# ppt0011/distributed_training

Hardware: AMD Instinct MI355X
Metric: images/sec (node) ResNet-50 at 1/2/4/8 MI355X; grad-sync bus GB/s (higher is better)
Workload: dtype bf16

## Files before the change

distributed_training_amd/_lib.py:

```python
from __future__ import annotations

import ctypes
import os
import threading

import torch

LIB_PATH = os.environ.get(
    "GSYNC_LIB", os.path.join(os.path.dirname(os.path.abspath(__file__)), "lib", "libgsync.so")
)

GS_OK = 0
GS_EINVAL, GS_EHIP, GS_ERCCL, GS_ESTATE, GS_ENOMEM, GS_ENODEV = -1, -2, -3, -4, -5, -6
GS_F32, GS_BF16, GS_F16, GS_F64, GS_I64, GS_I32, GS_U8 = 0, 1, 2, 3, 4, 5, 6
GS_DEV_HOST, GS_DEV_HIP = 0, 1
GS_SUM, GS_PROD, GS_MAX, GS_MIN, GS_AVG = 0, 1, 2, 3, 4
GS_SCALE_NONE, GS_SCALE_MUL, GS_SCALE_DIV = 0, 1, 2
GS_PLAN_SLOTS = 5
GS_RED_GROUPS = 64
GS_RED_PARTIALS = 1024
GS_BKT_AUTO_COLLECTIVE = 1
GS_BKT_GRAD_VIEW = 2
GS_BKT_NO_SCALE = 4
GS_BKT_REDUCE_SCATTER = 8
GS_BKT_NO_UNPACK = 16
GS_LAYOUT_NCHW, GS_LAYOUT_NHWC = 0, 1
GS_OP_PACK, GS_OP_UNPACK, GS_OP_SCALE, GS_OP_SQNORM, GS_OP_UNSCALE, GS_OP_SGD, GS_OP_ADAM, GS_OP_SUM = 1, 2, 3, 4, 5, 6, 7, 8
GS_OP_LARS_NORM, GS_OP_LARS = 9, 10
GS_OP_LAMB_MOMENTS, GS_OP_LAMB = 11, 12
GS_OP_EMA = 13
GS_EMA_EMA, GS_EMA_SWA, GS_EMA_WARMUP = 0, 1, 2

_TORCH_TO_GS = {
    torch.float32: GS_F32,
    torch.bfloat16: GS_BF16,
    torch.float16: GS_F16,
    torch.float64: GS_F64,
    torch.int64: GS_I64,
    torch.int32: GS_I32,
    torch.uint8: GS_U8,
}

_c_int, _c_i64, _c_f, _c_d, _vp = ctypes.c_int, ctypes.c_int64, ctypes.c_float, ctypes.c_double, ctypes.c_void_p
_p_i64 = ctypes.POINTER(ctypes.c_int64)
_p_i32 = ctypes.POINTER(ctypes.c_int32)
_p_u8 = ctypes.POINTER(ctypes.c_uint8)
_p_vp = ctypes.POINTER(ctypes.c_void_p)
_p_f = ctypes.POINTER(ctypes.c_float)

SIGNATURES = {
    "gs_version": (_c_int, []),
    "gs_last_error": (ctypes.c_char_p, []),
    "gs_device_count": (_c_int, []),
    "gs_set_host_threads": (_c_int, [_c_int]),
    "gs_comm_unique_id_bytes": (_c_int, []),
    "gs_comm_get_unique_id": (_c_int, [_p_u8]),
    "gs_comm_create": (_c_int, [_c_int, _c_int, _p_u8, _c_int, _p_vp]),
    "gs_comm_create_ex": (_c_int, [_c_int, _c_int, _p_u8, _c_int, _c_int, _p_vp]),
    "gs_comm_destroy": (_c_int, [_vp]),
    "gs_comm_abort": (_c_int, [_vp]),
    "gs_comm_set_timeout": (_c_int, [_vp, _c_i64]),
    "gs_comm_status": (_c_int, [_vp, ctypes.c_char_p, _c_int]),
    "gs_comm_rank": (_c_int, [_vp]),
    "gs_comm_world": (_c_int, [_vp]),
    "gs_comm_stream": (_c_int, [_vp, _p_vp]),
    "gs_stream_wait": (_c_int, [_vp, _vp]),
    "gs_allreduce": (_c_int, [_vp, _vp, _vp, _c_i64, _c_int, _c_int, _vp]),
    "gs_reduce_scatter": (_c_int, [_vp, _vp, _vp, _c_i64, _c_int, _c_int, _vp]),
    "gs_all_gather": (_c_int, [_vp, _vp, _vp, _c_i64, _c_int, _vp]),
    "gs_broadcast": (_c_int, [_vp, _vp, _vp, _c_i64, _c_int, _c_int, _vp]),
    "gs_allreduce_marked": (_c_int, [_vp, _vp, _vp, _c_i64, _c_int, _c_int, _vp, _vp]),
    "gs_all_gather_marked": (_c_int, [_vp, _vp, _vp, _c_i64, _c_int, _vp, _vp]),
    "gs_plan_create": (_c_int, [_c_int, _c_int, _c_int, _p_i64, _c_i64, _p_vp]),
    "gs_plan_create_ex": (_c_int, [_c_int, _c_int, _c_int, _p_i64, _c_i64, _c_i64, _p_vp]),
    "gs_plan_destroy": (_c_int, [_vp]),
    "gs_plan_flat_numel": (_c_i64, [_vp]),
    "gs_plan_offsets": (_c_int, [_vp, _p_i64]),
    "gs_plan_n_tasks": (_c_int, [_vp]),
    "gs_plan_task_units": (_c_i64, [_vp]),
    "gs_plan_set_hyper_source": (_c_int, [_vp, _vp]),
    "gs_watchdog_pause": (_c_int, [_c_int]),
    "gs_adam_hyper": (_c_int, [_c_int, _vp, _vp, _c_d, _c_d, _c_d, _vp, _vp, _vp]),
    "gs_plan_timer_enable": (_c_int, [_vp, _c_int]),
    "gs_plan_timer_read": (_c_int, [_vp, _p_f, _p_i32, _c_int]),
    "gs_plan_set_ptrs": (_c_int, [_vp, _c_int, _p_vp, _vp]),
    "gs_pack": (_c_int, [_vp, _c_int, _c_int, _vp, _c_int, _c_f, _c_int, _vp]),
    "gs_unpack": (_c_int, [_vp, _vp, _c_int, _c_int, _c_int, _vp, _c_int, _vp]),
    "gs_unpack_check": (_c_int, [_vp, _vp, _c_int, _c_int, _c_int, _vp, _vp]),
    "gs_scale": (_c_int, [_vp, _c_int, _c_int, _c_f, _c_int, _vp]),
    "gs_sqnorm": (_c_int, [_vp, _c_int, _c_int, _vp, _c_int, _vp]),
    "gs_sum": (_c_int, [_vp, _c_int, _c_int, _vp, _c_int, _vp]),
    "gs_sqnorm_partial": (_c_int, [_vp, _c_int, _c_int, _vp]),
    "gs_plan_set_clip": (_c_int, [_vp, _vp, _c_f, _c_f, _c_f, _c_f, _vp]),
    "gs_plan_set_read_hint": (_c_int, [_vp, _c_int]),
    "gs_sqnorm_partial_out": (_c_int, [_vp, _c_int, _c_int, _vp, _p_i32, _vp]),
    "gs_plan_set_clip_groups": (_c_int, [_vp, _vp, ctypes.c_int32, _c_f, _c_f, _c_f, _c_f, _vp]),
    "gs_clip_scale": (_c_int, [_vp, _c_int, _c_int, _vp]),
    "gs_rng_state_bytes": (_c_int, []),
    "gs_rng_draw_u32": (_c_int, [_vp, _c_i64, _c_i64, _vp]),
    "gs_randperm": (_c_int, [ctypes.c_uint64, _c_i64, _vp]),
    "gs_distributed_sampler_indices": (_c_int, [_c_i64, _c_int, _c_int, _c_int, ctypes.c_uint64, _c_i64, _c_int,
                                                _vp, _c_i64, _p_i64]),
    "gs_crop_flip_params": (_c_int, [_vp, _c_i64, _c_int, _c_int, _c_int, _c_int, _c_int, _c_int, _vp, _c_i64,
                                     _vp]),
    "gs_image_augment": (_c_int, [_c_int, _c_int, _vp, _vp, _c_i64, _c_int, _c_int, _c_int, _c_int, _c_int, _c_int,
                                  _vp, _c_i64, _vp, _c_int, _c_int, _vp, _vp]),
    "gs_bn_bwd_partials": (_c_int, [_c_i64, _c_int]),
    "gs_bn_bwd_reduce": (_c_int, [_vp, _vp, _vp, _vp, _vp, _vp, _c_i64, _c_i64, _c_int, _vp]),
    "gs_bn_bwd_reduce_fork": (_c_int, [_vp, _vp, _vp, _vp, _vp, _vp, _vp, _c_i64, _c_i64, _c_int, _vp]),
    "gs_bn_bwd_dx": (_c_int, [_vp, _vp, _vp, _vp, _vp, _vp, _vp, _c_i64, _vp, _vp, _vp, _c_i64, _c_int, _vp]),
    "gs_add_relu_fwd": (_c_int, [_vp, _vp, _c_i64, _vp]),
    "gs_relu_maxpool_fwd": (_c_int, [_vp, _vp, _vp, _c_i64, _c_int, _c_int, _c_int, _vp]),
    "gs_maxpool_bwd": (_c_int, [_vp, _vp, _vp, _vp, _c_i64, _c_int, _c_int, _c_int, _vp]),
    "gs_bn_infer_act": (_c_int, [_vp, _vp, _vp, _vp, _vp, _vp, _c_d, _c_int, _vp, _c_i64, _c_int, _vp]),
    "gs_bn_infer_relu_maxpool": (_c_int, [_vp, _vp, _vp, _vp, _vp, _c_d, _vp, _c_i64, _c_int, _c_int, _c_int, _vp]),
    "gs_eval_accumulate": (_c_int, [_c_int, _vp, _c_int, _vp, _c_i64, _c_i64, _c_i64, _c_i64, _p_i32, _c_int, _c_i64,
                                    _vp, _vp, _vp]),
    "gs_clip_coef":(_c_int, [_c_int, _vp, _c_f, _c_f, _vp, _vp, _vp]),
    "gs_unscale_check": (_c_int, [_vp, _c_int, _c_int, _vp, _vp, _vp]),
    "gs_sgd_step": (
        _c_int,
        [_vp, _c_int, _c_int, _c_d, _c_d, _c_d, _c_d, _c_int, _c_int, _c_int, _vp, _vp, _vp],
    ),
    "gs_adam_step": (
        _c_int,
        [_vp, _c_int, _c_int, _c_d, _c_d, _c_d, _c_d, _c_d, _c_int, _c_int, _c_d, _c_d, _vp, _vp, _vp],
    ),
    "gs_plan_set_adapt": (_c_int, [_vp, _p_i32]),
    "gs_lars_norms": (_c_int, [_vp, _c_int, _vp, _vp]),
    "gs_lars_step": (_c_int, [_vp, _c_int, _c_d, _c_d, _c_d, _c_d, _c_d, _vp, _vp, _vp, _vp]),
    "gs_lars_step_lowp": (_c_int, [_vp, _c_int, _c_int, _c_d, _c_d, _c_d, _c_d, _c_d, _vp, _vp, _vp, _vp]),
    "gs_lamb_step_lowp": (_c_int, [_vp, _c_int, _c_d, _c_d, _c_d, _c_d, _c_d, _c_d, _c_d, _vp, _vp, _vp]),
    "gs_lamb_moments": (_c_int, [_vp, _c_int, _c_d, _c_d, _c_d, _c_d, _c_d, _c_d, _vp, _vp, _vp, _vp]),
    "gs_lamb_step": (_c_int, [_vp, _c_d, _c_d, _c_d, _c_d, _c_d, _c_d, _c_d, _vp, _vp, _vp]),
    "gs_lamb_hyper": (_c_int, [_c_int, _vp, _vp, _c_d, _c_d, _c_int, _vp, _vp, _vp]),
    "gs_ema_step": (_c_int, [_vp, _c_int, _c_int, _c_d, _c_int, _vp]),
    "gs_ema_hyper": (_c_int, [_c_int, _vp, _c_int, _c_d, _vp, _vp]),
    "gs_compute_bucket_assignment": (
        _c_int,
        [_c_int, _p_i64, _p_i32, _p_i32, _c_int, _p_i64, _p_i32, _p_i32, _p_i32],
    ),
    "gs_bucketer_create": (
        _c_int,
        [_vp, _c_int, _c_int, _c_int, _p_i64, _c_int, _c_int, _p_i32, _p_i32, _c_int, _c_i64, _c_f, _c_int, _p_vp],
    ),
    "gs_bucketer_destroy": (_c_int, [_vp]),
    "gs_bucketer_bucket_numel": (_c_int, [_vp, _c_int, _p_i64]),
    "gs_bucketer_shard_numel": (_c_int, [_vp, _c_int, _p_i64]),
    "gs_bucketer_param_location": (_c_int, [_vp, _c_int, _p_i32, _p_i64]),
    "gs_bucketer_set_bucket_buffer": (_c_int, [_vp, _c_int, _vp]),
    "gs_bucketer_set_shard_buffer": (_c_int, [_vp, _c_int, _vp]),
    "gs_bucketer_prepare": (_c_int, [_vp, _vp]),
    "gs_bucketer_mark_ready": (_c_int, [_vp, _c_int, _vp, _vp, _p_i32, _p_i32]),
    "gs_bucketer_mark_unused": (_c_int, [_vp, _vp, _p_i32, _p_i32]),
    "gs_bucketer_finalize": (_c_int, [_vp, _vp]),
    "gs_bucketer_unpack_bucket": (_c_int, [_vp, _c_int, _vp]),
    "gs_bucketer_set_found_inf": (_c_int, [_vp, _vp]),
    "gs_bucketer_set_div_factor": (_c_int, [_vp, _c_f]),
    "gs_bucketer_set_debug": (_c_int, [_vp, _vp]),
    "gs_bucketer_set_bucket_dtype": (_c_int, [_vp, _c_int, _c_int, _c_int]),
    "gs_bucketer_last_comm_ms": (_c_int, [_vp, _c_int, _p_f]),
    "gs_bucketer_last_timing": (_c_int, [_vp, _c_int, _p_f]),
    "gs_bucketer_set_timeline": (_c_int, [_vp, _c_int]),
    "gs_bucketer_bucket_stream": (_c_int, [_vp, _c_int, ctypes.POINTER(_vp)]),
    "gs_bucketer_set_mark_consumer": (_c_int, [_vp, _vp]),
    "gs_bucketer_first_pack_plan": (_c_int, [_vp, _p_vp]),
}


class GsyncError(RuntimeError):
    """A libgsync entry point returned an error (message from gs_last_error)."""


class GsyncUnavailable(GsyncError):
    """libgsync.so is missing or failed to load."""


_lock = threading.Lock()
_lib = None
_load_error: str | None = None


def _load():
    global _lib, _load_error
    with _lock:
        if _lib is not None or _load_error is not None:
            return
        if not os.path.exists(LIB_PATH):
            _load_error = (
                f"libgsync not built: {LIB_PATH} is missing "
                "(run `python -c 'import __graft_entry__ as g; g.build()'` or `make -C distributed_training_amd/csrc`)"
            )
            return
        try:
            lib = ctypes.CDLL(LIB_PATH)
        except OSError as e:
            _load_error = f"failed to load {LIB_PATH}: {e}"
            return
        for name, (res, args) in SIGNATURES.items():
            fn = getattr(lib, name)
            fn.restype = res
            fn.argtypes = args
        _lib = lib


def lib():
    if _lib is None:
        _load()
        if _lib is None:
            raise GsyncUnavailable(_load_error)
    return _lib


def available() -> bool:
    try:
        lib()
        return True
    except GsyncUnavailable:
        return False


HOOK_PATH = os.path.join(os.path.dirname(os.path.abspath(LIB_PATH)), "_gshook.so")
if not os.path.exists(HOOK_PATH):
    HOOK_PATH = os.path.join(os.path.dirname(os.path.abspath(__file__)), "lib", "_gshook.so")
_hook_mod = None
_hook_error: str | None = None


def hook_module():
    global _hook_mod, _hook_error
    if _hook_mod is not None or _hook_error is not None:
        return _hook_mod
    lib()
    if os.path.realpath(LIB_PATH) != os.path.realpath(os.path.join(os.path.dirname(HOOK_PATH), "libgsync.so")):
        _hook_error = f"GSYNC_LIB={LIB_PATH} is not the library _gshook links"
        return None
    if not os.path.exists(HOOK_PATH):
        _hook_error = f"{HOOK_PATH} is not built"
        return None
    import importlib.util

    spec = importlib.util.spec_from_file_location("_gshook", HOOK_PATH)
    mod = importlib.util.module_from_spec(spec)
    spec.loader.exec_module(mod)
    _hook_mod = mod
    return mod


def check(rc: int, what: str = "") -> int:
    if rc < 0:
        msg = lib().gs_last_error().decode(errors="replace")
        raise GsyncError(f"{what or 'libgsync'} failed ({rc}): {msg}")
    return rc


def gs_dtype(dtype: torch.dtype) -> int:
    try:
        return _TORCH_TO_GS[dtype]
    except KeyError:
        raise TypeError(f"libgsync: unsupported dtype {dtype}") from None


def device_kind(t: torch.Tensor) -> int:
    if t.device.type == "cuda":
        return GS_DEV_HIP
    if t.device.type == "cpu":
        return GS_DEV_HOST
    raise TypeError(f"libgsync: unsupported device {t.device}")


def i64_array(vals):
    arr = (ctypes.c_int64 * max(1, len(vals)))(*vals)
    return arr


def i32_array(vals):
    return (ctypes.c_int32 * max(1, len(vals)))(*vals)


def ptr_array(vals):
    return (ctypes.c_void_p * max(1, len(vals)))(*vals)


def stream_ptr(device: torch.device) -> int | None:
    if device.type != "cuda":
        return None
    return torch.cuda.current_stream(device).cuda_stream


_deferred: list = []


def _capturing() -> bool:
    try:
        return torch.cuda.is_available() and torch.cuda.is_current_stream_capturing()
    except Exception:
        return False


def destroy(fn_name: str, handle) -> None:
    if _capturing():
        _deferred.append((fn_name, handle))
        return
    getattr(lib(), fn_name)(handle)


def flush_deferred() -> None:
    if not _deferred or _capturing():
        return
    while _deferred:
        fn_name, h = _deferred.pop(0)
        getattr(lib(), fn_name)(h)
```

distributed_training_amd/csrc/gs_bn_kernels.hip:

```cpp
#include <hip/hip_runtime.h>

#include <algorithm>
#include <climits>
#include <cmath>

#include "gs_common.h"

#ifndef GS_BN_NT
#define GS_BN_NT 0
#endif
#ifndef GS_BN_DX_RNE
#define GS_BN_DX_RNE 0
#endif

namespace gs {
namespace {

#define HIP_RET(expr)                                                               \
  do {                                                                              \
    hipError_t _e = (expr);                                                         \
    if (_e != hipSuccess)                                                           \
      return fail(GS_EHIP, std::string(#expr " failed: ") + hipGetErrorString(_e)); \
  } while (0)

typedef uint32_t bu4 __attribute__((ext_vector_type(4)));
typedef float bf4 __attribute__((ext_vector_type(4)));

constexpr int kBnTileVecs = 8;
constexpr int kBnMaxP = 512;
constexpr int kBnTargetBlocks = 1024;
constexpr int kBnUnroll = 4;
#ifndef GS_BN_FORK_UNROLL
#define GS_BN_FORK_UNROLL 4
#endif
constexpr int kBnForkUnroll = GS_BN_FORK_UNROLL;

struct BnGeom {
  int tx_log2;
  int ctiles;
  int P;
  int64_t rpb;
};

BnGeom bn_geom(int64_t R, int C) {
  const int V = C / 8;
  int l2 = 0;
  while ((1 << l2) < V && (1 << l2) < kBnTileVecs) ++l2;
  const int tx = 1 << l2, ty = kBlock / tx;
  const int64_t ctiles = (V + tx - 1) / tx;
  int64_t P = std::min<int64_t>(kBnMaxP, (R + ty - 1) / ty);
  P = std::min<int64_t>(P, static_cast<int64_t>(std::sqrt(0.5 * static_cast<double>(R))));
  P = std::min<int64_t>(P, kBnTargetBlocks / ctiles);
  P = std::max<int64_t>(P, 1);
  if (ctiles * P > 256) {
    const int64_t step = 256 / std::min<int64_t>(256, ctiles & -ctiles);
    if (P >= step) P -= P % step;
  }
  const int64_t rpb = (R + P - 1) / P;
  P = (R + rpb - 1) / rpb;
  return BnGeom{l2, static_cast<int>(ctiles), static_cast<int>(P), rpb};
}

__device__ __forceinline__ uint32_t to_bf16(float f) {
  uint32_t u = __float_as_uint(f);
  if ((u & 0x7fffffffu) > 0x7f800000u) return 0x7FC0u;
  return (u + 0x7FFFu + ((u >> 16) & 1u)) >> 16;
}

__device__ __forceinline__ void unpack8(const bu4& v, float (&f)[8]) {
#pragma unroll
  for (int i = 0; i < 4; ++i) {
    f[2 * i] = __uint_as_float(v[i] << 16);
    f[2 * i + 1] = __uint_as_float(v[i] & 0xffff0000u);
  }
}

__device__ __forceinline__ bu4 pack8_exact(const float (&f)[8]) {
  bu4 v;
#pragma unroll
  for (int i = 0; i < 4; ++i) v[i] = (__float_as_uint(f[2 * i]) >> 16) | (__float_as_uint(f[2 * i + 1]) & 0xffff0000u);
  return v;
}

__device__ __forceinline__ uint32_t to_bf16_trunc(float f) {
  uint32_t u = __float_as_uint(f);
  if ((~u & 0x7f800000u) == 0 && (u & 0xffffu) != 0) u |= 0x10000u;
  return u >> 16;
}

__device__ __forceinline__ bu4 pack8_dx(const float (&f)[8]) {
  bu4 v;
#pragma unroll
  for (int i = 0; i < 4; ++i) {
    if constexpr (GS_BN_DX_RNE) v[i] = to_bf16(f[2 * i]) | (to_bf16(f[2 * i + 1]) << 16);
    else v[i] = to_bf16_trunc(f[2 * i]) | (to_bf16_trunc(f[2 * i + 1]) << 16);
  }
  return v;
}

template <bool NT>
__device__ __forceinline__ bu4 ld16(const uint16_t* p) {
  const bu4* q = reinterpret_cast<const bu4*>(p);
  if constexpr (NT) return __builtin_nontemporal_load(q);
  else return *q;
}

__device__ __forceinline__ void st16(uint16_t* p, const bu4& v) { *reinterpret_cast<bu4*>(p) = v; }

__device__ __forceinline__ void relu_mask(float (&g)[8], const bu4& yv) {
  float yf[8];
  unpack8(yv, yf);
#pragma unroll
  for (int i = 0; i < 8; ++i) g[i] = yf[i] <= 0.f ? 0.f : g[i];
}

__device__ __forceinline__ void fork_sum(float (&g)[8], const bu4& bv) {
  float b[8];
  unpack8(bv, b);
#pragma unroll
  for (int i = 0; i < 8; ++i) g[i] = __uint_as_float(to_bf16(g[i] + b[i]) << 16);
}

template <bool RELU, bool WRITE_G, bool FORK>
__global__ void __launch_bounds__(kBlock)
bn_bwd_reduce_kernel(const uint16_t* __restrict__ x, const uint16_t* __restrict__ dy, const uint16_t* __restrict__ dy2,
                     const uint16_t* __restrict__ y, uint16_t* __restrict__ gout, const float* __restrict__ mean,
                     float* __restrict__ ws, int64_t R, int C, int tx_log2, int64_t rpb) {
  constexpr int U = FORK ? kBnForkUnroll : kBnUnroll;
  __shared__ float s_red[kBlock * 16];
  __shared__ double s_grp[kBlock];
  const int t = threadIdx.x;
  const int tx = 1 << tx_log2, ty = kBlock >> tx_log2;
  const int tx_i = t & (tx - 1), ty_i = t >> tx_log2;
  const int v = blockIdx.x * tx + tx_i;
  const bool active = v < (C >> 3);
  const int c0 = v * 8;
  const int64_t r0 = static_cast<int64_t>(blockIdx.y) * rpb;
  const int64_t r1 = std::min<int64_t>(R, r0 + rpb);

  float sg[8], sq[8], m[8];
#pragma unroll
  for (int i = 0; i < 8; ++i) {
    sg[i] = 0.f;
    sq[i] = 0.f;
    m[i] = active ? mean[c0 + i] : 0.f;
  }
  auto body = [&](const bu4& xv, const bu4& dv, const bu4& bv, const bu4& yv, int64_t off) {
    float xf[8], g[8];
    unpack8(xv, xf);
    unpack8(dv, g);
    if constexpr (FORK) fork_sum(g, bv);
    if constexpr (RELU) relu_mask(g, yv);
    if constexpr (WRITE_G) st16(gout + off, pack8_exact(g));
#pragma unroll
    for (int i = 0; i < 8; ++i) {
      sg[i] += g[i];
      sq[i] = fmaf(g[i], xf[i] - m[i], sq[i]);
    }
  };
  if (active) {
    const int64_t step = static_cast<int64_t>(ty) * C;
    int64_t r = r0 + ty_i;
    int64_t off = r * C + c0;
    for (; r + (U - 1) * ty < r1; r += U * ty, off += U * step) {
      bu4 xv[U], dv[U], bv[U] = {}, yv[U] = {};
#pragma unroll
      for (int k = 0; k < U; ++k) {
        xv[k] = ld16<false>(x + off + k * step);
        dv[k] = ld16<GS_BN_NT && WRITE_G>(dy + off + k * step);
        if constexpr (FORK) bv[k] = ld16<GS_BN_NT>(dy2 + off + k * step);
        if constexpr (RELU) yv[k] = ld16<GS_BN_NT && WRITE_G>(y + off + k * step);
      }
#pragma unroll
      for (int k = 0; k < U; ++k) body(xv[k], dv[k], bv[k], yv[k], off + k * step);
    }
    for (; r < r1; r += ty, off += step) {
      bu4 bv = {0u, 0u, 0u, 0u}, yv = {0u, 0u, 0u, 0u};
      const bu4 xv = ld16<false>(x + off), dv = ld16<false>(dy + off);
      if constexpr (FORK) bv = ld16<false>(dy2 + off);
      if constexpr (RELU) yv = ld16<false>(y + off);
      body(xv, dv, bv, yv, off);
    }
  }
  const int F = 16 << tx_log2;
#pragma unroll
  for (int i = 0; i < 8; ++i) {
    s_red[t * 16 + 2 * i] = sg[i];
    s_red[t * 16 + 2 * i + 1] = sq[i];
  }
  __syncthreads();
  {
    const int o = t & (F - 1), grp = t >> (tx_log2 + 4);
    double a = 0.0;
#pragma unroll
    for (int k = 0; k < 16; ++k) a += static_cast<double>(s_red[(grp * 16 + k) * F + o]);
    s_grp[t] = a;
  }
  __syncthreads();
  if (t < F) {
    const int G = kBlock / F;
    double a = 0.0;
    for (int k = 0; k < G; ++k) a += s_grp[k * F + t];
    const int ch = blockIdx.x * (tx * 8) + (t >> 1);
    if (ch < C) ws[(static_cast<int64_t>(blockIdx.y) * C + ch) * 2 + (t & 1)] = static_cast<float>(a);
  }
}

template <bool RELU>
__global__ void __launch_bounds__(kBlock)
bn_bwd_dx_kernel(const uint16_t* __restrict__ x, const uint16_t* __restrict__ dy, const uint16_t* __restrict__ y,
                 const float* __restrict__ mean, const float* __restrict__ invstd, const float* __restrict__ weight,
                 const float* __restrict__ ws, int P, uint16_t* __restrict__ dx, float* __restrict__ gw,
                 float* __restrict__ gb, int64_t R, int C, int tx_log2, int64_t rpb, double inv_R) {
  __shared__ double s_fold[kBlock * 4];
  __shared__ double s_sum[16 * kBnTileVecs];
  const int t = threadIdx.x;
  const int tx = 1 << tx_log2, ty = kBlock >> tx_log2;
  const int tx_i = t & (tx - 1), ty_i = t >> tx_log2;
  const int tile_c0 = blockIdx.x * (tx * 8);
  {
    const int F4 = 4 << tx_log2, G4 = kBlock / F4;
    const int q = t & (F4 - 1), grp = t >> (tx_log2 + 2);
    double a[4] = {0.0, 0.0, 0.0, 0.0};
    if (tile_c0 + 2 * q < C) {
      const bf4* base = reinterpret_cast<const bf4*>(ws + static_cast<int64_t>(tile_c0) * 2) + q;
      const int64_t stride = C >> 1;
#pragma unroll 8
      for (int p = grp; p < P; p += G4) {
        const bf4 w4 = base[p * stride];
#pragma unroll
        for (int j = 0; j < 4; ++j) a[j] += static_cast<double>(w4[j]);
      }
    }
#pragma unroll
    for (int j = 0; j < 4; ++j) s_fold[t * 4 + j] = a[j];
    __syncthreads();
    if (t < 4 * F4) {
      double b = 0.0;
      for (int k = 0; k < G4; ++k) b += s_fold[k * 4 * F4 + t];
      s_sum[t] = b;
    }
    __syncthreads();
  }
  if (blockIdx.y == 0 && t < tx * 8 && tile_c0 + t < C) {
    gb[tile_c0 + t] = static_cast<float>(s_sum[2 * t]);
    gw[tile_c0 + t] = static_cast<float>(static_cast<double>(invstd[tile_c0 + t]) * s_sum[2 * t + 1]);
  }
  const int v = blockIdx.x * tx + tx_i;
  if (v >= (C >> 3)) return;
  const int c0 = v * 8;
  float m[8], a[8], m1[8], k2[8];
#pragma unroll
  for (int i = 0; i < 8; ++i) {
    const float is = invstd[c0 + i];
    m[i] = mean[c0 + i];
    a[i] = weight[c0 + i] * is;
    m1[i] = static_cast<float>(s_sum[tx_i * 16 + 2 * i] * inv_R);
    k2[i] = static_cast<float>(static_cast<double>(is) * is * s_sum[tx_i * 16 + 2 * i + 1] * inv_R);
  }
  auto body = [&](const bu4& xv, const bu4& dv, const bu4& yv, int64_t off) {
    float xf[8], g[8];
    unpack8(xv, xf);
    unpack8(dv, g);
    if constexpr (RELU) relu_mask(g, yv);
#pragma unroll
    for (int i = 0; i < 8; ++i) g[i] = a[i] * fmaf(m[i] - xf[i], k2[i], g[i] - m1[i]);
    st16(dx + off, pack8_dx(g));
  };
  const int64_t r0 = static_cast<int64_t>(blockIdx.y) * rpb;
  const int64_t r1 = std::min<int64_t>(R, r0 + rpb);
  const int64_t step = static_cast<int64_t>(ty) * C;
  int64_t r = r0 + ty_i;
  int64_t off = r * C + c0;
  for (; r + (kBnUnroll - 1) * ty < r1; r += kBnUnroll * ty, off += kBnUnroll * step) {
    bu4 xv[kBnUnroll], dv[kBnUnroll], yv[kBnUnroll] = {};
#pragma unroll
    for (int k = 0; k < kBnUnroll; ++k) {
      xv[k] = ld16<GS_BN_NT>(x + off + k * step);
      dv[k] = ld16<GS_BN_NT>(dy + off + k * step);
      if constexpr (RELU) yv[k] = ld16<GS_BN_NT>(y + off + k * step);
    }
#pragma unroll
    for (int k = 0; k < kBnUnroll; ++k) body(xv[k], dv[k], yv[k], off + k * step);
  }
  for (; r < r1; r += ty, off += step) {
    bu4 yv = {0u, 0u, 0u, 0u};
    const bu4 xv = ld16<false>(x + off), dv = ld16<false>(dy + off);
    if constexpr (RELU) yv = ld16<false>(y + off);
    body(xv, dv, yv, off);
  }
}

__global__ void __launch_bounds__(kBlock)
add_relu_fwd_kernel(uint16_t* __restrict__ t, const uint16_t* __restrict__ id, int64_t nvec) {
  const int64_t base = static_cast<int64_t>(blockIdx.x) * (kBlock * kBnUnroll) + threadIdx.x;
  bu4 a[kBnUnroll], b[kBnUnroll];
#pragma unroll
  for (int k = 0; k < kBnUnroll; ++k) {
    const int64_t i = base + k * kBlock;
    if (i < nvec) {
      a[k] = ld16<false>(t + i * 8);
      b[k] = ld16<false>(id + i * 8);
    }
  }
#pragma unroll
  for (int k = 0; k < kBnUnroll; ++k) {
    const int64_t i = base + k * kBlock;
    if (i < nvec) {
      float af[8], bf[8];
      unpack8(a[k], af);
      unpack8(b[k], bf);
#pragma unroll
      for (int j = 0; j < 8; ++j) {
        const float s = __uint_as_float(to_bf16(af[j] + bf[j]) << 16);
        af[j] = s != s ? s : fmaxf(s, 0.f);
      }
      st16(t + i * 8, pack8_exact(af));
    }
  }
}


__device__ __forceinline__ float relu1(float v) { return v > 0.f ? v : (v != v ? v : 0.f); }

__global__ void __launch_bounds__(kBlock)
relu_maxpool_fwd_kernel(const uint16_t* __restrict__ y, uint16_t* __restrict__ pooled, uint8_t* __restrict__ idx,
                        int64_t nvec, int H, int W, int OH, int OW, int V) {
  const int64_t i = static_cast<int64_t>(blockIdx.x) * kBlock + threadIdx.x;
  if (i >= nvec) return;
  const int cv = static_cast<int>(i % V);
  int64_t p = i / V;
  const int ow = static_cast<int>(p % OW);
  p /= OW;
  const int oh = static_cast<int>(p % OH);
  const int64_t n = p / OH;
  const int h0 = 2 * oh - 1, w0 = 2 * ow - 1;
  const int64_t C = static_cast<int64_t>(V) * 8;
  bu4 in[9];
  bool ok[9];
#pragma unroll
  for (int kh = 0; kh < 3; ++kh) {
#pragma unroll
    for (int kw = 0; kw < 3; ++kw) {
      const int ih = h0 + kh, iw = w0 + kw, k = 3 * kh + kw;
      ok[k] = ih >= 0 && ih < H && iw >= 0 && iw < W;
      in[k] = bu4{0u, 0u, 0u, 0u};
      if (ok[k]) in[k] = ld16<false>(y + ((n * H + ih) * W + iw) * C + cv * 8);
    }
  }
  float best[8];
  uint32_t code[8];
#pragma unroll
  for (int j = 0; j < 8; ++j) {
    best[j] = -INFINITY;
    code[j] = 0;
  }
#pragma unroll
  for (int k = 0; k < 9; ++k) {
    float f[8];
    unpack8(in[k], f);
#pragma unroll
    for (int j = 0; j < 8; ++j) {
      const float v = relu1(f[j]);
      const bool take = ok[k] && (v > best[j] || v != v);
      best[j] = take ? v : best[j];
      code[j] = take ? static_cast<uint32_t>(k) : code[j];
    }
  }
  st16(pooled + i * 8, pack8_exact(best));
  uint2 c;
  c.x = code[0] | (code[1] << 8) | (code[2] << 16) | (code[3] << 24);
  c.y = code[4] | (code[5] << 8) | (code[6] << 16) | (code[7] << 24);
  *reinterpret_cast<uint2*>(idx + i * 8) = c;
}

template <bool FORK>
__global__ void __launch_bounds__(kBlock)
maxpool_bwd_kernel(const uint16_t* __restrict__ da, const uint16_t* __restrict__ db, const uint8_t* __restrict__ idx,
                   uint16_t* __restrict__ dx, int64_t nquad, int H, int W, int OH, int OW, int V) {
  const int64_t i = static_cast<int64_t>(blockIdx.x) * kBlock + threadIdx.x;
  if (i >= nquad) return;
  const int cv = static_cast<int>(i % V);
  int64_t p = i / V;
  const int b = static_cast<int>(p % OW);
  p /= OW;
  const int a = static_cast<int>(p % OH);
  const int64_t n = p / OH;
  const bool more_h = a + 1 < OH, more_w = b + 1 < OW;
  uint2 cw[4];
  int64_t ovec[4];
  bool ok[4];
#pragma unroll
  for (int k = 0; k < 4; ++k) {
    const int al = k >> 1, be = k & 1;
    ok[k] = (al == 0 || more_h) && (be == 0 || more_w);
    ovec[k] = ((n * OH + a + al) * OW + b + be) * V + cv;
    cw[k] = uint2{0xffffffffu, 0xffffffffu};
    if (ok[k]) cw[k] = *reinterpret_cast<const uint2*>(idx + ovec[k] * 8);
  }
  auto has = [](const uint2& w, uint32_t c) {
    const uint32_t x0 = w.x ^ (c * 0x01010101u), x1 = w.y ^ (c * 0x01010101u);
    return ((((x0 - 0x01010101u) & ~x0) | ((x1 - 0x01010101u) & ~x1)) & 0x80808080u) != 0;
  };
  bool hit[4];
  hit[0] = true;
  hit[1] = ok[1] && (has(cw[1], 3u) || has(cw[1], 6u));
  hit[2] = ok[2] && (has(cw[2], 1u) || has(cw[2], 2u));
  hit[3] = ok[3] && has(cw[3], 0u);
  bu4 av[4], bv[4];
#pragma unroll
  for (int k = 0; k < 4; ++k) {
    av[k] = bv[k] = bu4{0u, 0u, 0u, 0u};
    if (hit[k]) {
      av[k] = ld16<false>(da + ovec[k] * 8);
      if constexpr (FORK) bv[k] = ld16<false>(db + ovec[k] * 8);
    }
  }
  const bool many = H * W > 1;
  float acc[4][8];
#pragma unroll
  for (int q = 0; q < 4; ++q)
#pragma unroll
    for (int j = 0; j < 8; ++j) acc[q][j] = 0.f;
#pragma unroll
  for (int k = 0; k < 4; ++k) {
    const int al = k >> 1, be = k & 1;
    float g[8];
    unpack8(av[k], g);
    if constexpr (FORK) fork_sum(g, bv[k]);
#pragma unroll
    for (int q = 0; q < 4; ++q) {
      const int dh = q >> 1, dw = q & 1;
      if (dh < al || dw < be) continue;
      const uint32_t want = static_cast<uint32_t>(3 * (dh + 1 - 2 * al) + (dw + 1 - 2 * be));
      const bool single = many && !(dh == 1 && more_h) && !(dw == 1 && more_w);
#pragma unroll
      for (int j = 0; j < 8; ++j) {
        const uint32_t cj = ((j < 4 ? cw[k].x : cw[k].y) >> (8 * (j & 3))) & 0xffu;
        const bool m = hit[k] && cj == want;
        acc[q][j] = m ? (single ? g[j] : acc[q][j] + g[j]) : acc[q][j];
      }
    }
  }
  const int64_t C = static_cast<int64_t>(V) * 8;
#pragma unroll
  for (int q = 0; q < 4; ++q) {
    const int ih = 2 * a + (q >> 1), iw = 2 * b + (q & 1);
    if (ih < H && iw < W) {
      bu4 out;
#pragma unroll
      for (int r = 0; r < 4; ++r) out[r] = to_bf16(acc[q][2 * r]) | (to_bf16(acc[q][2 * r + 1]) << 16);
      st16(dx + ((n * H + ih) * W + iw) * C + cv * 8, out);
    }
  }
}

constexpr int kBnInferBlocks = 2048;
#ifndef GS_BN_INFER_TILE_VECS
#define GS_BN_INFER_TILE_VECS 32
#endif
constexpr int kBnInferTileVecs = GS_BN_INFER_TILE_VECS;

BnGeom bn_infer_geom(int64_t R, int C) {
  const int V = C / 8;
  int l2 = 0;
  while ((1 << l2) < V && (1 << l2) < kBnInferTileVecs) ++l2;
  const int tx = 1 << l2, ty = kBlock / tx;
  const int64_t ctiles = (V + tx - 1) / tx;
  const int64_t per = static_cast<int64_t>(ty) * kBnUnroll;
  int64_t P = std::min<int64_t>((R + per - 1) / per, std::max<int64_t>(1, kBnInferBlocks / ctiles));
  P = std::max<int64_t>(P, 1);
  const int64_t rpb = (R + P - 1) / P;
  P = (R + rpb - 1) / rpb;
  return BnGeom{l2, static_cast<int>(ctiles), static_cast<int>(P), rpb};
}

__device__ __forceinline__ void infer_affine(const float* __restrict__ rm, const float* __restrict__ rv,
                                             const float* __restrict__ w, const float* __restrict__ b, float eps,
                                             int c0, float (&s)[8], float (&t)[8]) {
  const bf4 m0 = *reinterpret_cast<const bf4*>(rm + c0), m1 = *reinterpret_cast<const bf4*>(rm + c0 + 4);
  const bf4 v0 = *reinterpret_cast<const bf4*>(rv + c0), v1 = *reinterpret_cast<const bf4*>(rv + c0 + 4);
  const bf4 w0 = *reinterpret_cast<const bf4*>(w + c0), w1 = *reinterpret_cast<const bf4*>(w + c0 + 4);
  const bf4 b0 = *reinterpret_cast<const bf4*>(b + c0), b1 = *reinterpret_cast<const bf4*>(b + c0 + 4);
#pragma unroll
  for (int i = 0; i < 8; ++i) {
    const float m = i < 4 ? m0[i & 3] : m1[i & 3], v = i < 4 ? v0[i & 3] : v1[i & 3];
    const float wi = i < 4 ? w0[i & 3] : w1[i & 3], bi = i < 4 ? b0[i & 3] : b1[i & 3];
    s[i] = wi * (1.0f / sqrtf(v + eps));
    t[i] = fmaf(-m, s[i], bi);
  }
}

__device__ __forceinline__ bu4 pack8_rne(const float (&f)[8]) {
  bu4 v;
#pragma unroll
  for (int i = 0; i < 4; ++i) v[i] = to_bf16(f[2 * i]) | (to_bf16(f[2 * i + 1]) << 16);
  return v;
}

template <bool RES, bool RELU>
__global__ void __launch_bounds__(kBlock)
bn_infer_act_kernel(const uint16_t* x, const uint16_t* __restrict__ res, const float* __restrict__ rm,
                    const float* __restrict__ rv, const float* __restrict__ w, const float* __restrict__ b, float eps,
                    uint16_t* y, int64_t R, int C, int tx_log2, int64_t rpb) {
  const int t_ = threadIdx.x;
  const int tx = 1 << tx_log2, ty = kBlock >> tx_log2;
  const int tx_i = t_ & (tx - 1), ty_i = t_ >> tx_log2;
  const int v = blockIdx.x * tx + tx_i;
  if (v >= (C >> 3)) return;
  const int c0 = v * 8;
  const int64_t r0 = static_cast<int64_t>(blockIdx.y) * rpb;
  const int64_t r1 = std::min<int64_t>(R, r0 + rpb);
  const int64_t step = static_cast<int64_t>(ty) * C;
  int64_t r = r0 + ty_i;
  int64_t off = r * C + c0;
  float s[8], t[8];
  infer_affine(rm, rv, w, b, eps, c0, s, t);
  auto body = [&](const bu4& xv, const bu4& rvv, int64_t off) {
    float f[8], r[8];
    unpack8(xv, f);
    if constexpr (RES) unpack8(rvv, r);
#pragma unroll
    for (int i = 0; i < 8; ++i) {
      float a = fmaf(f[i], s[i], t[i]);
      if constexpr (RES) a = a + r[i];
      if constexpr (RELU) a = relu1(a);
      f[i] = a;
    }
    st16(y + off, pack8_rne(f));
  };
  for (; r + (kBnUnroll - 1) * ty < r1; r += kBnUnroll * ty, off += kBnUnroll * step) {
    bu4 xv[kBnUnroll], rr[kBnUnroll] = {};
#pragma unroll
    for (int k = 0; k < kBnUnroll; ++k) {
      xv[k] = ld16<GS_BN_NT>(x + off + k * step);
      if constexpr (RES) rr[k] = ld16<false>(res + off + k * step);
    }
#pragma unroll
    for (int k = 0; k < kBnUnroll; ++k) body(xv[k], rr[k], off + k * step);
  }
  for (; r < r1; r += ty, off += step) {
    bu4 rr = {0u, 0u, 0u, 0u};
    const bu4 xv = ld16<false>(x + off);
    if constexpr (RES) rr = ld16<false>(res + off);
    body(xv, rr, off);
  }
}

__global__ void __launch_bounds__(kBlock)
bn_infer_relu_maxpool_kernel(const uint16_t* __restrict__ x, const float* __restrict__ rm,
                             const float* __restrict__ rv, const float* __restrict__ w, const float* __restrict__ b,
                             float eps, uint16_t* __restrict__ pooled, int64_t OR, int H, int W, int OH, int OW, int C,
                             int tx_log2, int64_t rpb) {
  const int t_ = threadIdx.x;
  const int tx = 1 << tx_log2, ty = kBlock >> tx_log2;
  const int tx_i = t_ & (tx - 1), ty_i = t_ >> tx_log2;
  const int v = blockIdx.x * tx + tx_i;
  if (v >= (C >> 3)) return;
  const int c0 = v * 8;
  float s[8], t[8];
  infer_affine(rm, rv, w, b, eps, c0, s, t);
  const int64_t r0 = static_cast<int64_t>(blockIdx.y) * rpb;
  const int64_t r1 = std::min<int64_t>(OR, r0 + rpb);
  for (int64_t p = r0 + ty_i; p < r1; p += ty) {
    const int ow = static_cast<int>(p % OW);
    const int64_t q = p / OW;
    const int oh = static_cast<int>(q % OH);
    const int64_t n = q / OH;
    const int h0 = 2 * oh - 1, w0 = 2 * ow - 1;
    bu4 in[9];
    bool ok[9];
#pragma unroll
    for (int kh = 0; kh < 3; ++kh) {
#pragma unroll
      for (int kw = 0; kw < 3; ++kw) {
        const int ih = h0 + kh, iw = w0 + kw, k = 3 * kh + kw;
        ok[k] = ih >= 0 && ih < H && iw >= 0 && iw < W;
        in[k] = bu4{0u, 0u, 0u, 0u};
        if (ok[k]) in[k] = ld16<false>(x + ((n * H + ih) * W + iw) * C + c0);
      }
    }
    float best[8];
#pragma unroll
    for (int j = 0; j < 8; ++j) best[j] = -INFINITY;
#pragma unroll
    for (int k = 0; k < 9; ++k) {
      float f[8];
      unpack8(in[k], f);
#pragma unroll
      for (int j = 0; j < 8; ++j) {
        const float a = __uint_as_float(to_bf16(relu1(fmaf(f[j], s[j], t[j]))) << 16);
        const bool take = ok[k] && (a > best[j] || a != a);
        best[j] = take ? a : best[j];
      }
    }
    st16(pooled + p * C + c0, pack8_exact(best));
  }
}

bool aligned16(const void* p) { return (reinterpret_cast<uintptr_t>(p) & 15u) == 0; }

int check_shape(int64_t R, int C) {
  GS_CHECK_ARG(R > 0 && C > 0 && C % 8 == 0, "bn: R > 0, C > 0 and C % 8 == 0 required");
  GS_CHECK_ARG(R <= (INT64_MAX / 4) / C, "bn: R * C too large");
  return GS_OK;
}

}
}

using namespace gs;

extern "C" int gs_bn_bwd_partials(int64_t R, int C) {
  GS_TRY_RET(check_shape(R, C));
  return bn_geom(R, C).P;
}

namespace gs {
namespace {

bool overlap(const void* p, int64_t pbytes, const void* q, int64_t qbytes) {
  if (!p || !q) return false;
  const uintptr_t a = reinterpret_cast<uintptr_t>(p), b = reinterpret_cast<uintptr_t>(q);
  return a < b + static_cast<uintptr_t>(qbytes) && b < a + static_cast<uintptr_t>(pbytes);
}
bool overlap(const void* p, const void* q, int64_t bytes) { return overlap(p, bytes, q, bytes); }

struct PoolGeom {
  int OH, OW;
  int64_t in_vecs, out_vecs;
};

int pool_geom(const std::string& w, int64_t N, int H, int W, int C, PoolGeom* g) {
  GS_CHECK_ARG(N > 0 && H > 0 && W > 0 && C > 0 && C % 8 == 0, w + ": N, H, W, C > 0 and C % 8 == 0 required");
  GS_CHECK_ARG(N <= ((INT64_MAX / 4) / C / H) / W, w + ": N * H * W * C too large");
  g->OH = (H - 1) / 2 + 1;
  g->OW = (W - 1) / 2 + 1;
  g->in_vecs = N * H * W * (C / 8);
  g->out_vecs = N * g->OH * g->OW * (C / 8);
  GS_CHECK_ARG((g->in_vecs + kBlock - 1) / kBlock <= INT_MAX, w + ": N * H * W * C too large");
  return GS_OK;
}

int bn_reduce(const char* who, const void* x, const void* dy, const void* dy_b, const void* y, void* g_out,
              const float* mean, float* ws, int64_t ws_floats, int64_t R, int C, void* stream) {
  const std::string w(who);
  GS_TRY_RET(check_shape(R, C));
  GS_CHECK_ARG(x && dy && mean && ws, w + ": null pointer");
  GS_CHECK_ARG(!g_out || y || dy_b, w + ": g_out needs y");
  GS_CHECK_ARG(!dy_b || g_out, w + ": two gradients need g_out");
  GS_CHECK_ARG(aligned16(x) && aligned16(dy) && aligned16(dy_b) && aligned16(y) && aligned16(g_out) && aligned16(ws),
               w + ": pointers must be 16-byte aligned");
  if (dy_b) {
    const int64_t bytes = R * C * 2;
    GS_CHECK_ARG(!overlap(g_out, x, bytes) && !overlap(g_out, dy, bytes) && !overlap(g_out, dy_b, bytes) &&
                     !overlap(g_out, y, bytes),
                 w + ": g_out overlaps an input");
  }
  const BnGeom g = bn_geom(R, C);
  GS_CHECK_ARG(ws_floats >= static_cast<int64_t>(g.P) * C * 2, w + ": workspace too small");
  const dim3 grid(g.ctiles, g.P), block(kBlock);
  hipStream_t s = static_cast<hipStream_t>(stream);
  const uint16_t* xp = static_cast<const uint16_t*>(x);
  const uint16_t* dp = static_cast<const uint16_t*>(dy);
  const uint16_t* bp = static_cast<const uint16_t*>(dy_b);
  const uint16_t* yp = static_cast<const uint16_t*>(y);
  uint16_t* gp = static_cast<uint16_t*>(g_out);
#define GS_BN_REDUCE(RELU, WRITE_G, FORK)                                                                        \
  hipLaunchKernelGGL((bn_bwd_reduce_kernel<RELU, WRITE_G, FORK>), grid, block, 0, s, xp, dp, bp, yp, gp, mean, ws, R, \
                     C, g.tx_log2, g.rpb)
  if (bp && yp) GS_BN_REDUCE(true, true, true);
  else if (bp) GS_BN_REDUCE(false, true, true);
  else if (gp) GS_BN_REDUCE(true, true, false);
  else if (yp) GS_BN_REDUCE(true, false, false);
  else GS_BN_REDUCE(false, false, false);
#undef GS_BN_REDUCE
  HIP_RET(hipGetLastError());
  return GS_OK;
}

}
}

extern "C" int gs_bn_bwd_reduce(const void* x, const void* dy, const void* y, void* g_out, const float* mean,
                                float* ws, int64_t ws_floats, int64_t R, int C, void* stream) {
  return bn_reduce("gs_bn_bwd_reduce", x, dy, nullptr, y, g_out, mean, ws, ws_floats, R, C, stream);
}

extern "C" int gs_bn_bwd_reduce_fork(const void* x, const void* dy_a, const void* dy_b, const void* y, void* g_out,
                                     const float* mean, float* ws, int64_t ws_floats, int64_t R, int C,
                                     void* stream) {
  return bn_reduce("gs_bn_bwd_reduce_fork", x, dy_a, dy_b, y, g_out, mean, ws, ws_floats, R, C, stream);
}

extern "C" int gs_bn_bwd_dx(const void* x, const void* dy, const void* y, const float* mean, const float* invstd,
                            const float* weight, const float* ws, int64_t ws_floats, void* dx, float* grad_weight,
                            float* grad_bias, int64_t R, int C, void* stream) {
  GS_TRY_RET(check_shape(R, C));
  GS_CHECK_ARG(x && dy && mean && invstd && weight && ws && dx && grad_weight && grad_bias,
               "gs_bn_bwd_dx: null pointer");
  GS_CHECK_ARG(aligned16(x) && aligned16(dy) && aligned16(y) && aligned16(dx) && aligned16(ws),
               "gs_bn_bwd_dx: pointers must be 16-byte aligned");
  const BnGeom g = bn_geom(R, C);
  GS_CHECK_ARG(ws_floats >= static_cast<int64_t>(g.P) * C * 2, "gs_bn_bwd_dx: workspace too small");
  const dim3 grid(g.ctiles, g.P), block(kBlock);
  hipStream_t s = static_cast<hipStream_t>(stream);
  const uint16_t* xp = static_cast<const uint16_t*>(x);
  const uint16_t* dp = static_cast<const uint16_t*>(dy);
  const uint16_t* yp = static_cast<const uint16_t*>(y);
  uint16_t* op = static_cast<uint16_t*>(dx);
  const double inv_R = 1.0 / static_cast<double>(R);
  if (yp)
    hipLaunchKernelGGL((bn_bwd_dx_kernel<true>), grid, block, 0, s, xp, dp, yp, mean, invstd, weight, ws, g.P, op,
                       grad_weight, grad_bias, R, C, g.tx_log2, g.rpb, inv_R);
  else
    hipLaunchKernelGGL((bn_bwd_dx_kernel<false>), grid, block, 0, s, xp, dp, yp, mean, invstd, weight, ws, g.P, op,
                       grad_weight, grad_bias, R, C, g.tx_log2, g.rpb, inv_R);
  HIP_RET(hipGetLastError());
  return GS_OK;
}

extern "C" int gs_add_relu_fwd(void* t, const void* identity, int64_t n, void* stream) {
  GS_CHECK_ARG(t && identity && n > 0 && n % 8 == 0, "gs_add_relu_fwd: n > 0, n % 8 == 0 and pointers required");
  GS_CHECK_ARG(aligned16(t) && aligned16(identity), "gs_add_relu_fwd: pointers must be 16-byte aligned");
  const int64_t nvec = n / 8;
  const int64_t blocks = (nvec + kBlock * kBnUnroll - 1) / (kBlock * kBnUnroll);
  GS_CHECK_ARG(blocks <= INT_MAX, "gs_add_relu_fwd: n too large");
  hipLaunchKernelGGL(add_relu_fwd_kernel, dim3(static_cast<unsigned>(blocks)), dim3(kBlock), 0,
                     static_cast<hipStream_t>(stream), static_cast<uint16_t*>(t),
                     static_cast<const uint16_t*>(identity), nvec);
  HIP_RET(hipGetLastError());
  return GS_OK;
}

extern "C" int gs_relu_maxpool_fwd(const void* y, void* pooled, void* idx, int64_t N, int H, int W, int C,
                                   void* stream) {
  const std::string w("gs_relu_maxpool_fwd");
  PoolGeom g;
  GS_TRY_RET(pool_geom(w, N, H, W, C, &g));
  GS_CHECK_ARG(y && pooled && idx, w + ": null pointer");
  GS_CHECK_ARG(aligned16(y) && aligned16(pooled) && aligned16(idx), w + ": pointers must be 16-byte aligned");
  const int64_t ib = g.in_vecs * 16, ob = g.out_vecs * 16, xb = g.out_vecs * 8;
  GS_CHECK_ARG(!overlap(y, ib, pooled, ob) && !overlap(y, ib, idx, xb) && !overlap(pooled, ob, idx, xb),
               w + ": buffers overlap");
  const unsigned blocks = static_cast<unsigned>((g.out_vecs + kBlock - 1) / kBlock);
  hipLaunchKernelGGL(relu_maxpool_fwd_kernel, dim3(blocks), dim3(kBlock), 0, static_cast<hipStream_t>(stream),
                     static_cast<const uint16_t*>(y), static_cast<uint16_t*>(pooled), static_cast<uint8_t*>(idx),
                     g.out_vecs, H, W, g.OH, g.OW, C / 8);
  HIP_RET(hipGetLastError());
  return GS_OK;
}

extern "C" int gs_maxpool_bwd(const void* d_a, const void* d_b, const void* idx, void* dx, int64_t N, int H, int W,
                              int C, void* stream) {
  const std::string w("gs_maxpool_bwd");
  PoolGeom g;
  GS_TRY_RET(pool_geom(w, N, H, W, C, &g));
  GS_CHECK_ARG(d_a && idx && dx, w + ": null pointer");
  GS_CHECK_ARG(aligned16(d_a) && aligned16(d_b) && aligned16(idx) && aligned16(dx),
               w + ": pointers must be 16-byte aligned");
  const int64_t ib = g.in_vecs * 16, ob = g.out_vecs * 16, xb = g.out_vecs * 8;
  GS_CHECK_ARG(!overlap(dx, ib, d_a, ob) && !overlap(dx, ib, d_b, ob) && !overlap(dx, ib, idx, xb),
               w + ": dx overlaps an input");
  const dim3 grid(static_cast<unsigned>((g.out_vecs + kBlock - 1) / kBlock)), block(kBlock);
  hipStream_t s = static_cast<hipStream_t>(stream);
  const uint16_t* ap = static_cast<const uint16_t*>(d_a);
  const uint16_t* bp = static_cast<const uint16_t*>(d_b);
  const uint8_t* ip = static_cast<const uint8_t*>(idx);
  uint16_t* op = static_cast<uint16_t*>(dx);
  if (bp)
    hipLaunchKernelGGL((maxpool_bwd_kernel<true>), grid, block, 0, s, ap, bp, ip, op, g.out_vecs, H, W, g.OH, g.OW,
                       C / 8);
  else
    hipLaunchKernelGGL((maxpool_bwd_kernel<false>), grid, block, 0, s, ap, bp, ip, op, g.out_vecs, H, W, g.OH, g.OW,
                       C / 8);
  HIP_RET(hipGetLastError());
  return GS_OK;
}

extern "C" int gs_bn_infer_act(const void* x, const void* residual, const float* running_mean,
                               const float* running_var, const float* weight, const float* bias, double eps, int relu,
                               void* y, int64_t R, int C, void* stream) {
  const std::string w("gs_bn_infer_act");
  GS_TRY_RET(check_shape(R, C));
  GS_CHECK_ARG(x && running_mean && running_var && weight && bias && y, w + ": null pointer");
  GS_CHECK_ARG(eps >= 0.0 && eps == eps, w + ": eps must be >= 0");
  GS_CHECK_ARG(aligned16(x) && aligned16(residual) && aligned16(y) && aligned16(running_mean) &&
                   aligned16(running_var) && aligned16(weight) && aligned16(bias),
               w + ": pointers must be 16-byte aligned");
  const int64_t bytes = R * C * 2;
  GS_CHECK_ARG(x == y || !overlap(x, y, bytes), w + ": y overlaps x without being x");
  GS_CHECK_ARG(!overlap(residual, y, bytes), w + ": y overlaps the residual");
  const BnGeom g = bn_infer_geom(R, C);
  const dim3 grid(g.ctiles, g.P), block(kBlock);
  hipStream_t s = static_cast<hipStream_t>(stream);
  const uint16_t* xp = static_cast<const uint16_t*>(x);
  const uint16_t* rp = static_cast<const uint16_t*>(residual);
  uint16_t* yp = static_cast<uint16_t*>(y);
  const float e = static_cast<float>(eps);
#define GS_BN_INFER(RES, RELU)                                                                                   \
  hipLaunchKernelGGL((bn_infer_act_kernel<RES, RELU>), grid, block, 0, s, xp, rp, running_mean, running_var, weight, \
                     bias, e, yp, R, C, g.tx_log2, g.rpb)
  if (rp && relu) GS_BN_INFER(true, true);
  else if (rp) GS_BN_INFER(true, false);
  else if (relu) GS_BN_INFER(false, true);
  else GS_BN_INFER(false, false);
#undef GS_BN_INFER
  HIP_RET(hipGetLastError());
  return GS_OK;
}

extern "C" int gs_bn_infer_relu_maxpool(const void* x, const float* running_mean, const float* running_var,
                                        const float* weight, const float* bias, double eps, void* pooled, int64_t N,
                                        int H, int W, int C, void* stream) {
  const std::string w("gs_bn_infer_relu_maxpool");
  PoolGeom pg;
  GS_TRY_RET(pool_geom(w, N, H, W, C, &pg));
  GS_CHECK_ARG(x && running_mean && running_var && weight && bias && pooled, w + ": null pointer");
  GS_CHECK_ARG(eps >= 0.0 && eps == eps, w + ": eps must be >= 0");
  GS_CHECK_ARG(aligned16(x) && aligned16(pooled) && aligned16(running_mean) && aligned16(running_var) &&
                   aligned16(weight) && aligned16(bias),
               w + ": pointers must be 16-byte aligned");
  GS_CHECK_ARG(!overlap(x, pg.in_vecs * 16, pooled, pg.out_vecs * 16), w + ": buffers overlap");
  const int64_t OR = N * pg.OH * pg.OW;
  const BnGeom g = bn_infer_geom(OR, C);
  hipLaunchKernelGGL(bn_infer_relu_maxpool_kernel, dim3(g.ctiles, g.P), dim3(kBlock), 0,
                     static_cast<hipStream_t>(stream), static_cast<const uint16_t*>(x), running_mean, running_var,
                     weight, bias, static_cast<float>(eps), static_cast<uint16_t*>(pooled), OR, H, W, pg.OH, pg.OW, C,
                     g.tx_log2, g.rpb);
  HIP_RET(hipGetLastError());
  return GS_OK;
}
```

distributed_training_amd/fused_bn.py:

```python
from __future__ import annotations

import contextlib
import os

import torch
import torch.nn.functional as F
from torch.autograd.function import once_differentiable

from . import _lib as L

last_path: str | None = None

_CL = torch.channels_last
_partials: dict = {}


def _n_partials(R: int, C: int) -> int:
    P = _partials.get((R, C))
    if P is None:
        P = _partials[(R, C)] = L.check(L.lib().gs_bn_bwd_partials(R, C), "gs_bn_bwd_partials")
    return P


def _eligible(bn, x, relu, residual) -> bool:
    return bn.training and _shape_eligible(bn, x, relu, residual)


def _shape_eligible(bn, x, relu, residual) -> bool:
    if os.environ.get("GSYNC_FUSED_BN", "1") == "0":
        return False
    if not (x.is_cuda and x.dim() == 4 and x.dtype == torch.bfloat16 and x.numel() > 0):
        return False
    w, b = bn.weight, bn.bias
    if w is None or b is None or w.dtype != torch.float32 or b.dtype != torch.float32:
        return False
    if x.shape[1] % 8 != 0 or not x.is_contiguous(memory_format=_CL):
        return False
    if bn._forward_pre_hooks or bn._forward_hooks:
        return False
    if residual is not None and not (relu and residual.shape == x.shape and residual.dtype == x.dtype
                                     and residual.device == x.device and residual.is_contiguous(memory_format=_CL)):
        return False
    return L.available()


_fused_eval = False


@contextlib.contextmanager
def fused_eval(enabled: bool = True):
    global _fused_eval
    prev, _fused_eval = _fused_eval, bool(enabled)
    try:
        yield
    finally:
        _fused_eval = prev


def _eval_eligible(bn, x, relu, residual) -> bool:
    if not _fused_eval or bn.training:
        return False
    rm, rv = bn.running_mean, bn.running_var
    if rm is None or rv is None or rm.dtype != torch.float32 or rv.dtype != torch.float32:
        return False
    if not _shape_eligible(bn, x, relu, residual):
        return False
    if torch.is_grad_enabled() and (x.requires_grad or bn.weight.requires_grad or bn.bias.requires_grad
                                    or (residual is not None and residual.requires_grad)):
        return False
    ptrs = [x.data_ptr(), rm.data_ptr(), rv.data_ptr(), bn.weight.data_ptr(), bn.bias.data_ptr()]
    if residual is not None:
        ptrs.append(residual.data_ptr())
    return all(p % 16 == 0 for p in ptrs)


def _infer_act(bn, x, relu, residual):
    y = torch.empty_like(x)
    C = x.shape[1]
    L.check(L.lib().gs_bn_infer_act(x.data_ptr(), None if residual is None else residual.data_ptr(),
                                    bn.running_mean.data_ptr(), bn.running_var.data_ptr(), bn.weight.data_ptr(),
                                    bn.bias.data_ptr(), bn.eps, int(bool(relu)), y.data_ptr(), x.numel() // C, C,
                                    L.stream_ptr(x.device)), "gs_bn_infer_act")
    return y


def _infer_relu_pool(bn, x):
    N, C, H, W = x.shape
    out = torch.empty((N, C, (H - 1) // 2 + 1, (W - 1) // 2 + 1), dtype=x.dtype, device=x.device, memory_format=_CL)
    L.check(L.lib().gs_bn_infer_relu_maxpool(x.data_ptr(), bn.running_mean.data_ptr(), bn.running_var.data_ptr(),
                                             bn.weight.data_ptr(), bn.bias.data_ptr(), bn.eps, out.data_ptr(), N, H,
                                             W, C, L.stream_ptr(x.device)), "gs_bn_infer_relu_maxpool")
    return out


class _BnAct(torch.autograd.Function):
    @staticmethod
    def forward(ctx, x, weight, bias, residual, bn, momentum, relu, fork=False):
        y, mean, invstd, _, _ = torch._batch_norm_impl_index(
            x, weight, bias, bn.running_mean, bn.running_var, True, momentum, bn.eps, torch.backends.cudnn.enabled)
        if not y.is_contiguous(memory_format=_CL):
            raise RuntimeError("fused_bn: batch_norm returned a layout other than its channels_last input's")
        if residual is not None:
            L.check(L.lib().gs_add_relu_fwd(y.data_ptr(), residual.data_ptr(), y.numel(), L.stream_ptr(y.device)),
                    "gs_add_relu_fwd")
        elif relu:
            torch.relu_(y)
        ctx.relu = relu
        ctx.has_residual = residual is not None
        ctx.save_for_backward(x, weight, mean, invstd, y if relu else None)
        if fork:
            ctx.set_materialize_grads(False)
            return y, y.view_as(y)
        return y

    @staticmethod
    @once_differentiable
    def backward(ctx, dy, dy_b=None):
        x, weight, mean, invstd, y = ctx.saved_tensors
        if dy is None:
            dy, dy_b = dy_b, None
        if dy is None:
            return None, None, None, None, None, None, None, None
        if not dy.is_contiguous(memory_format=_CL):
            dy = dy.contiguous(memory_format=_CL)
        if dy_b is not None and not dy_b.is_contiguous(memory_format=_CL):
            dy_b = dy_b.contiguous(memory_format=_CL)
        C = x.shape[1]
        R = x.numel() // C
        ws = torch.empty(_n_partials(R, C) * C * 2, dtype=torch.float32, device=x.device)
        dx = torch.empty_like(x)
        gw = torch.empty_like(weight)
        gb = torch.empty_like(weight)
        lib, stream = L.lib(), L.stream_ptr(x.device)
        yp = y.data_ptr() if ctx.relu else None
        g = None
        if dy_b is not None:
            g = torch.empty_like(x)
            L.check(lib.gs_bn_bwd_reduce_fork(x.data_ptr(), dy.data_ptr(), dy_b.data_ptr(), yp, g.data_ptr(),
                                              mean.data_ptr(), ws.data_ptr(), ws.numel(), R, C, stream),
                    "gs_bn_bwd_reduce_fork")
            dy, yp = g, None
        elif ctx.has_residual:
            g = torch.empty_like(x)
            L.check(lib.gs_bn_bwd_reduce(x.data_ptr(), dy.data_ptr(), yp, g.data_ptr(), mean.data_ptr(),
                                         ws.data_ptr(), ws.numel(), R, C, stream), "gs_bn_bwd_reduce")
            dy, yp = g, None
        else:
            L.check(lib.gs_bn_bwd_reduce(x.data_ptr(), dy.data_ptr(), yp, None, mean.data_ptr(), ws.data_ptr(),
                                         ws.numel(), R, C, stream), "gs_bn_bwd_reduce")
        L.check(lib.gs_bn_bwd_dx(x.data_ptr(), dy.data_ptr(), yp, mean.data_ptr(), invstd.data_ptr(),
                                 weight.data_ptr(), ws.data_ptr(), ws.numel(), dx.data_ptr(), gw.data_ptr(),
                                 gb.data_ptr(), R, C, stream), "gs_bn_bwd_dx")
        return dx, gw, gb, g if ctx.has_residual else None, None, None, None, None


class _BnReluPool(torch.autograd.Function):

    @staticmethod
    def forward(ctx, x, weight, bias, bn, momentum, fork):
        y, mean, invstd, _, _ = torch._batch_norm_impl_index(
            x, weight, bias, bn.running_mean, bn.running_var, True, momentum, bn.eps, torch.backends.cudnn.enabled)
        if not y.is_contiguous(memory_format=_CL):
            raise RuntimeError("fused_bn: batch_norm returned a layout other than its channels_last input's")
        N, C, H, W = y.shape
        OH, OW = (H - 1) // 2 + 1, (W - 1) // 2 + 1
        out = torch.empty((N, C, OH, OW), dtype=y.dtype, device=y.device, memory_format=_CL)
        idx = torch.empty((N, OH, OW, C), dtype=torch.uint8, device=y.device)
        L.check(L.lib().gs_relu_maxpool_fwd(y.data_ptr(), out.data_ptr(), idx.data_ptr(), N, H, W, C,
                                            L.stream_ptr(y.device)), "gs_relu_maxpool_fwd")
        ctx.save_for_backward(x, weight, mean, invstd, y, idx)
        if fork:
            ctx.set_materialize_grads(False)
            return out, out.view_as(out)
        return out

    @staticmethod
    @once_differentiable
    def backward(ctx, d_a, d_b=None):
        x, weight, mean, invstd, y, idx = ctx.saved_tensors
        if d_a is None:
            d_a, d_b = d_b, None
        if d_a is None:
            return None, None, None, None, None, None
        if not d_a.is_contiguous(memory_format=_CL):
            d_a = d_a.contiguous(memory_format=_CL)
        if d_b is not None and not d_b.is_contiguous(memory_format=_CL):
            d_b = d_b.contiguous(memory_format=_CL)
        N, C, H, W = x.shape
        R = N * H * W
        lib, stream = L.lib(), L.stream_ptr(x.device)
        dy = torch.empty_like(x)
        L.check(lib.gs_maxpool_bwd(d_a.data_ptr(), None if d_b is None else d_b.data_ptr(), idx.data_ptr(),
                                   dy.data_ptr(), N, H, W, C, stream), "gs_maxpool_bwd")
        ws = torch.empty(_n_partials(R, C) * C * 2, dtype=torch.float32, device=x.device)
        dx = torch.empty_like(x)
        gw = torch.empty_like(weight)
        gb = torch.empty_like(weight)
        L.check(lib.gs_bn_bwd_reduce(x.data_ptr(), dy.data_ptr(), y.data_ptr(), None, mean.data_ptr(), ws.data_ptr(),
                                     ws.numel(), R, C, stream), "gs_bn_bwd_reduce")
        L.check(lib.gs_bn_bwd_dx(x.data_ptr(), dy.data_ptr(), y.data_ptr(), mean.data_ptr(), invstd.data_ptr(),
                                 weight.data_ptr(), ws.data_ptr(), ws.numel(), dx.data_ptr(), gw.data_ptr(),
                                 gb.data_ptr(), R, C, stream), "gs_bn_bwd_dx")
        return dx, gw, gb, None, None, None


def _bookkeeping(bn) -> float:
    momentum = 0.0 if bn.momentum is None else bn.momentum
    if bn.track_running_stats and bn.num_batches_tracked is not None:
        bn.num_batches_tracked.add_(1)
        if bn.momentum is None:
            momentum = 1.0 / float(bn.num_batches_tracked)
    return momentum


def _pool_eligible(pool) -> bool:
    def is_(v, k):
        return v == k or v == (k, k) or v == [k, k]

    return (type(pool) is torch.nn.MaxPool2d and is_(pool.kernel_size, 3) and is_(pool.stride, 2)
            and is_(pool.padding, 1) and is_(pool.dilation, 1) and not pool.ceil_mode and not pool.return_indices
            and not (pool._forward_pre_hooks or pool._forward_hooks))


def bn_relu_pool(bn, x, pool, fork: bool = True):
    global last_path
    if _pool_eligible(pool) and _eval_eligible(bn, x, True, None):
        last_path = "fused_eval"
        out = _infer_relu_pool(bn, x)
        return (out, out) if fork else out
    if _pool_eligible(pool) and _eligible(bn, x, True, None):
        momentum = _bookkeeping(bn)
        last_path = "fused"
        return _BnReluPool.apply(x, bn.weight, bn.bias, bn, momentum, fork)
    out = pool(bn_act(bn, x))
    return (out, out) if fork else out


def bn_act(bn, x, relu: bool = True, residual=None, fork: bool = False):
    global last_path
    if _eval_eligible(bn, x, relu, residual):
        last_path = "fused_eval"
        out = _infer_act(bn, x, relu, residual)
        return (out, out) if fork else out
    if _eligible(bn, x, relu, residual):
        momentum = _bookkeeping(bn)
        last_path = "fused"
        return _BnAct.apply(x, bn.weight, bn.bias, residual, bn, momentum, relu, fork)
    last_path = "stock"
    out = bn(x)
    if residual is not None:
        out += residual
    if relu:
        out = F.relu(out, inplace=True)
    return (out, out) if fork else out
```

include/gsync.h:

```cpp
#ifndef GSYNC_H
#define GSYNC_H

#include <stdint.h>

#ifdef __cplusplus
extern "C" {
#endif

#define GSYNC_VERSION 1000

#define GS_OK 0
#define GS_EINVAL (-1)
#define GS_EHIP (-2)
#define GS_ERCCL (-3)
#define GS_ESTATE (-4)
#define GS_ENOMEM (-5)
#define GS_ENODEV (-6)

#define GS_F32 0
#define GS_BF16 1
#define GS_F16 2
#define GS_F64 3
#define GS_I64 4
#define GS_I32 5
#define GS_U8 6

int gs_set_host_threads(int n);

#define GS_DEV_HOST 0
#define GS_DEV_HIP 1

#define GS_SUM 0
#define GS_PROD 1
#define GS_MAX 2
#define GS_MIN 3
#define GS_AVG 4

#define GS_SCALE_NONE 0
#define GS_SCALE_MUL 1
#define GS_SCALE_DIV 2

typedef struct gs_comm gs_comm;
typedef struct gs_plan gs_plan;
typedef struct gs_bucketer gs_bucketer;

int gs_version(void);
const char* gs_last_error(void);
int gs_device_count(void);

int gs_comm_unique_id_bytes(void);
int gs_comm_get_unique_id(uint8_t* out );
int gs_comm_create(int rank, int world, const uint8_t* uid, int device, gs_comm** out);
int gs_comm_create_ex(int rank, int world, const uint8_t* uid, int device, int max_ctas, gs_comm** out);
int gs_comm_destroy(gs_comm* c);
int gs_comm_abort(gs_comm* c);
int gs_comm_set_timeout(gs_comm* c, int64_t timeout_ms);
int gs_watchdog_pause(int pause);
int gs_comm_status(gs_comm* c, char* reason, int cap);
int gs_comm_rank(gs_comm* c);
int gs_comm_world(gs_comm* c);
int gs_comm_stream(gs_comm* c, void** stream_out);
int gs_stream_wait(void* waiter, void* signaler);

int gs_allreduce(gs_comm* c, const void* send, void* recv, int64_t count, int dtype, int op,
                 void* stream);
int gs_reduce_scatter(gs_comm* c, const void* send, void* recv, int64_t recv_count, int dtype,
                      int op, void* stream);
int gs_all_gather(gs_comm* c, const void* send, void* recv, int64_t send_count, int dtype,
                  void* stream);
int gs_allreduce_marked(gs_comm* c, const void* send, void* recv, int64_t count, int dtype, int op,
                        void* stream, gs_plan* consumer);
int gs_all_gather_marked(gs_comm* c, const void* send, void* recv, int64_t send_count, int dtype,
                         void* stream, gs_plan* consumer);
int gs_broadcast(gs_comm* c, const void* send, void* recv, int64_t count, int dtype, int root,
                 void* stream);

#define GS_PLAN_SLOTS 5
int gs_plan_create(int device_kind, int device, int n_tensors, const int64_t* numels,
                   int64_t align_elems, gs_plan** out);
int gs_plan_create_ex(int device_kind, int device, int n_tensors, const int64_t* numels,
                      int64_t align_elems, int64_t task_units, gs_plan** out);
int gs_plan_destroy(gs_plan* p);
int64_t gs_plan_flat_numel(gs_plan* p);
int gs_plan_offsets(gs_plan* p, int64_t* out );
int gs_plan_n_tasks(gs_plan* p);
int64_t gs_plan_task_units(gs_plan* p);
#define GS_OP_PACK 1
#define GS_OP_UNPACK 2
#define GS_OP_SCALE 3
#define GS_OP_SQNORM 4
#define GS_OP_UNSCALE 5
#define GS_OP_SGD 6
#define GS_OP_ADAM 7
#define GS_OP_SUM 8
#define GS_OP_LARS_NORM 9
#define GS_OP_LARS 10
#define GS_OP_LAMB_MOMENTS 11
#define GS_OP_LAMB 12
#define GS_OP_EMA 13
int gs_plan_timer_enable(gs_plan* p, int n_slots);
int gs_plan_timer_read(gs_plan* p, float* ms_out, int32_t* kind_out, int cap);
int gs_plan_set_ptrs(gs_plan* p, int slot, void* const* ptrs, void* stream);

int gs_pack(gs_plan* p, int src_slot, int src_dtype, void* flat, int flat_dtype, float scale,
            int scale_mode, void* stream);
int gs_unpack(gs_plan* p, const void* flat, int flat_dtype, int dst_slot, int dst_dtype,
              float* sqnorm_dev, int accumulate, void* stream);
int gs_unpack_check(gs_plan* p, const void* flat, int flat_dtype, int dst_slot, int dst_dtype,
                    float* found_inf, void* stream);
int gs_scale(gs_plan* p, int slot, int dtype, float s, int scale_mode, void* stream);
int gs_sqnorm(gs_plan* p, int slot, int dtype, float* sqnorm_dev, int accumulate, void* stream);
int gs_sum(gs_plan* p, int slot, int dtype, float* sum_dev, int accumulate, void* stream);
int gs_sqnorm_partial(gs_plan* p, int slot, int dtype, void* stream);
int gs_plan_set_read_hint(gs_plan* p, int hint);
int gs_plan_set_clip(gs_plan* p, const float* sqnorm_dev, float max_norm, float eps, float sq_mul,
                     float coef_mul, float* out_dev);
#define GS_RED_GROUPS 64
#define GS_RED_PARTIALS 1024
int gs_sqnorm_partial_out(gs_plan* p, int slot, int dtype, float* groups_out, int32_t* n_groups,
                          void* stream);
int gs_plan_set_clip_groups(gs_plan* p, const float* groups_dev, int32_t n_groups, float max_norm,
                            float eps, float sq_mul, float coef_mul, float* out_dev);
int gs_clip_scale(gs_plan* p, int slot, int dtype, void* stream);
int gs_clip_coef(int device_kind, const float* sqnorm_dev, float max_norm, float eps,
                 float* coef_dev, float* norm_dev, void* stream);
int gs_unscale_check(gs_plan* p, int slot, int dtype, const float* inv_scale_dev,
                     float* found_inf_dev, void* stream);

int gs_sgd_step(gs_plan* p, int grad_dtype, int lowp_dtype, double lr, double momentum,
                double dampening, double weight_decay, int nesterov, int maximize, int first_step,
                const float* grad_scale_dev, const float* found_inf_dev, void* stream);
int gs_adam_step(gs_plan* p, int grad_dtype, int lowp_dtype, double lr, double beta1,
                 double beta2, double eps, double weight_decay, int adamw, int maximize,
                 double step_size, double bias_correction2_sqrt, const float* grad_scale_dev,
                 const float* found_inf_dev, void* stream);
int gs_plan_set_adapt(gs_plan* p, const int32_t* adapt);
int gs_lars_norms(gs_plan* p, int grad_dtype, float* norms_out, void* stream);
int gs_lars_step(gs_plan* p, int grad_dtype, double lr, double momentum, double weight_decay,
                 double trust_coefficient, double eps, const float* norms,
                 const float* grad_scale_dev, const float* found_inf_dev, void* stream);
int gs_lars_step_lowp(gs_plan* p, int grad_dtype, int lowp_dtype, double lr, double momentum,
                      double weight_decay, double trust_coefficient, double eps, const float* norms,
                      const float* grad_scale_dev, const float* found_inf_dev, void* stream);
int gs_plan_set_hyper_source(gs_plan* p, const float* hyper);
int gs_adam_hyper(int device_kind, double* step, const double* lr, double beta1, double beta2,
                  double weight_decay, const float* found_inf, float* hyper, void* stream);
int gs_lamb_moments(gs_plan* p, int grad_dtype, double beta1, double beta2, double eps, double weight_decay,
                    double bc1, double bc2_sqrt, float* norms_out, const float* grad_scale_dev,
                    const float* found_inf_dev, void* stream);
int gs_lamb_step(gs_plan* p, double lr, double eps, double weight_decay, double bc1, double bc2_sqrt,
                 double min_ratio, double max_ratio, const float* norms, const float* found_inf_dev, void* stream);
int gs_lamb_step_lowp(gs_plan* p, int lowp_dtype, double lr, double eps, double weight_decay,
                      double bc1, double bc2_sqrt, double min_ratio, double max_ratio,
                      const float* norms, const float* found_inf_dev, void* stream);
int gs_lamb_hyper(int device_kind, double* step, const double* lr, double beta1, double beta2, int bias_correction,
                  const float* found_inf, float* hyper, void* stream);

int gs_ema_step(gs_plan* p, int src_dtype, int lowp_dtype , double weight, int copy,
                void* stream);
#define GS_EMA_EMA 0
#define GS_EMA_SWA 1
#define GS_EMA_WARMUP 2
int gs_ema_hyper(int device_kind, int64_t* n_averaged, int mode, double decay, float* hyper ,
                 void* stream);

int gs_compute_bucket_assignment(int n, const int64_t* nbytes, const int32_t* dtype_keys,
                                 const int32_t* order, int n_limits, const int64_t* limits,
                                 int32_t* bucket_of ,
                                 int32_t* bucket_members ,
                                 int32_t* bucket_counts );

#define GS_BKT_AUTO_COLLECTIVE 1
#define GS_BKT_GRAD_VIEW 2
#define GS_BKT_NO_SCALE 4
#define GS_BKT_REDUCE_SCATTER 8
#define GS_BKT_NO_UNPACK 16

int gs_bucketer_create(gs_comm* comm, int device_kind, int device, int n_params,
                       const int64_t* numels, int grad_dtype, int n_buckets,
                       const int32_t* bucket_counts, const int32_t* bucket_members,
                       int bucket_dtype, int64_t align_elems, float div_factor, int flags,
                       gs_bucketer** out);
int gs_bucketer_destroy(gs_bucketer* b);
int gs_bucketer_bucket_numel(gs_bucketer* b, int bucket, int64_t* out);
int gs_bucketer_shard_numel(gs_bucketer* b, int bucket, int64_t* out);
int gs_bucketer_param_location(gs_bucketer* b, int param, int32_t* bucket, int64_t* offset);
int gs_bucketer_set_bucket_dtype(gs_bucketer* b, int bucket, int grad_dtype, int bucket_dtype);
int gs_bucketer_set_bucket_buffer(gs_bucketer* b, int bucket, void* ptr);
int gs_bucketer_set_shard_buffer(gs_bucketer* b, int bucket, void* ptr);
int gs_bucketer_prepare(gs_bucketer* b, float* sqnorm_dev);
int gs_bucketer_mark_ready(gs_bucketer* b, int param, const void* grad, void* stream,
                           int32_t* ready_out, int32_t* n_ready);
int gs_bucketer_mark_unused(gs_bucketer* b, void* stream, int32_t* ready_out, int32_t* n_ready);
int gs_bucketer_finalize(gs_bucketer* b, void* stream);
int gs_bucketer_set_found_inf(gs_bucketer* b, float* found_inf);
int gs_bucketer_set_div_factor(gs_bucketer* b, float div_factor);
int gs_bucketer_unpack_bucket(gs_bucketer* b, int bucket, void* stream);
int gs_bucketer_set_mark_consumer(gs_bucketer* b, gs_plan* consumer);
int gs_bucketer_first_pack_plan(gs_bucketer* b, gs_plan** out);
int gs_bucketer_last_comm_ms(gs_bucketer* b, int bucket, float* ms);
int gs_bucketer_last_timing(gs_bucketer* b, int bucket, float* out );
int gs_bucketer_set_timeline(gs_bucketer* b, int level);
int gs_bucketer_bucket_stream(gs_bucketer* b, int bucket, void** stream);
int gs_bucketer_set_debug(gs_bucketer* b, float* sums);

#define GS_LAYOUT_NCHW 0
#define GS_LAYOUT_NHWC 1
int gs_rng_state_bytes(void);
int gs_rng_draw_u32(uint8_t* state, int64_t state_bytes, int64_t n, uint32_t* out);
int gs_randperm(uint64_t seed, int64_t n, int64_t* out);
int gs_distributed_sampler_indices(int64_t n, int num_replicas, int rank, int shuffle, uint64_t seed,
                                   int64_t epoch, int drop_last, int64_t* out, int64_t cap,
                                   int64_t* count);
int gs_crop_flip_params(const int64_t* indices, int64_t B, int in_h, int in_w, int pad, int out_h,
                        int out_w, int flip, uint8_t* rng_state, int64_t state_bytes,
                        int32_t* params );
int gs_image_augment(int device_kind, int device, const uint8_t* src, const int64_t* labels, int64_t n_src,
                     int H, int W, int C, int pad, int out_h, int out_w, const int32_t* params, int64_t B,
                     void* out, int out_dtype, int out_layout, int64_t* out_labels, void* stream);

int gs_bn_bwd_partials(int64_t R, int C);
int gs_bn_bwd_reduce(const void* x, const void* dy, const void* y, void* g_out, const float* mean, float* ws,
                     int64_t ws_floats, int64_t R, int C, void* stream);
int gs_bn_bwd_reduce_fork(const void* x, const void* dy_a, const void* dy_b, const void* y, void* g_out,
                          const float* mean, float* ws, int64_t ws_floats, int64_t R, int C, void* stream);
int gs_bn_bwd_dx(const void* x, const void* dy, const void* y, const float* mean, const float* invstd,
                 const float* weight, const float* ws, int64_t ws_floats, void* dx, float* grad_weight,
                 float* grad_bias, int64_t R, int C, void* stream);
int gs_add_relu_fwd(void* t, const void* identity, int64_t n, void* stream);
int gs_relu_maxpool_fwd(const void* y, void* pooled, void* idx, int64_t N, int H, int W, int C, void* stream);
int gs_maxpool_bwd(const void* d_a, const void* d_b, const void* idx, void* dx, int64_t N, int H, int W, int C,
                   void* stream);

int gs_bn_infer_act(const void* x, const void* residual, const float* running_mean, const float* running_var,
                    const float* weight, const float* bias, double eps, int relu, void* y, int64_t R, int C,
                    void* stream);
int gs_bn_infer_relu_maxpool(const void* x, const float* running_mean, const float* running_var, const float* weight,
                             const float* bias, double eps, void* pooled, int64_t N, int H, int W, int C,
                             void* stream);
int gs_eval_accumulate(int device_kind, const void* logits, int logits_dtype, const int64_t* labels, int64_t B,
                       int64_t K, int64_t row_stride, int64_t n_valid, const int32_t* topk, int n_topk,
                       int64_t ignore_index, void* ws, void* acc, void* stream);

#ifdef __cplusplus
}
#endif
#endif
```

Baseline: 6889.

## Save ReLU masks as packed bits and read them in BN backward

In the forward pass, the ReLU, add+ReLU and ReLU+maxpool kernels now also write a one-bit-per-element mask. The BN backward reduce and dx kernels read this mask instead of the full bf16 activation y. Each backward pass reads one mask byte per eight elements in place of 16 bytes, which cuts memory traffic in these bandwidth-bound kernels. The cost is an extra mask write in the forward pass and an extra mask buffer allocation, though autograd may no longer need to hold y. The reduce kernel also gets occupancy hints, and a GSYNC_BN_MASK env var (default on) selects the path.

```diff
diff --git a/distributed_training_amd/_lib.py b/distributed_training_amd/_lib.py
--- a/distributed_training_amd/_lib.py
+++ b/distributed_training_amd/_lib.py
@@ -112,6 +112,12 @@
     "gs_add_relu_fwd": (_c_int, [_vp, _vp, _c_i64, _vp]),
     "gs_relu_maxpool_fwd": (_c_int, [_vp, _vp, _vp, _c_i64, _c_int, _c_int, _c_int, _vp]),
     "gs_maxpool_bwd": (_c_int, [_vp, _vp, _vp, _vp, _c_i64, _c_int, _c_int, _c_int, _vp]),
+    "gs_relu_mask_fwd": (_c_int, [_vp, _vp, _c_i64, _vp]),
+    "gs_add_relu_mask_fwd": (_c_int, [_vp, _vp, _vp, _c_i64, _vp]),
+    "gs_relu_maxpool_mask_fwd": (_c_int, [_vp, _vp, _vp, _vp, _c_i64, _c_int, _c_int, _c_int, _vp]),
+    "gs_bn_bwd_reduce_bits": (_c_int, [_vp, _vp, _vp, _vp, _vp, _vp, _c_i64, _c_i64, _c_int, _vp]),
+    "gs_bn_bwd_reduce_fork_bits": (_c_int, [_vp, _vp, _vp, _vp, _vp, _vp, _vp, _c_i64, _c_i64, _c_int, _vp]),
+    "gs_bn_bwd_dx_bits": (_c_int, [_vp, _vp, _vp, _vp, _vp, _vp, _vp, _c_i64, _vp, _vp, _vp, _c_i64, _c_int, _vp]),
     "gs_bn_infer_act": (_c_int, [_vp, _vp, _vp, _vp, _vp, _vp, _c_d, _c_int, _vp, _c_i64, _c_int, _vp]),
     "gs_bn_infer_relu_maxpool": (_c_int, [_vp, _vp, _vp, _vp, _vp, _c_d, _vp, _c_i64, _c_int, _c_int, _c_int, _vp]),
     "gs_eval_accumulate": (_c_int, [_c_int, _vp, _c_int, _vp, _c_i64, _c_i64, _c_i64, _c_i64, _p_i32, _c_int, _c_i64,
diff --git a/distributed_training_amd/csrc/gs_bn_kernels.hip b/distributed_training_amd/csrc/gs_bn_kernels.hip
--- a/distributed_training_amd/csrc/gs_bn_kernels.hip
+++ b/distributed_training_amd/csrc/gs_bn_kernels.hip
@@ -114,6 +114,20 @@
   for (int i = 0; i < 8; ++i) g[i] = yf[i] <= 0.f ? 0.f : g[i];
 }
 
+enum : int { kMaskNone = 0, kMaskY = 1, kMaskBits = 2 };
+
+__device__ __forceinline__ void relu_mask_bits(float (&g)[8], uint32_t mb) {
+#pragma unroll
+  for (int i = 0; i < 8; ++i) g[i] = (mb >> i) & 1u ? g[i] : 0.f;
+}
+
+__device__ __forceinline__ uint8_t mask_byte(const float (&f)[8]) {
+  uint32_t mb = 0;
+#pragma unroll
+  for (int j = 0; j < 8; ++j) mb |= (f[j] <= 0.f ? 0u : 1u) << j;
+  return static_cast<uint8_t>(mb);
+}
+
 __device__ __forceinline__ void fork_sum(float (&g)[8], const bu4& bv) {
   float b[8];
   unpack8(bv, b);
@@ -121,11 +135,12 @@
   for (int i = 0; i < 8; ++i) g[i] = __uint_as_float(to_bf16(g[i] + b[i]) << 16);
 }
 
-template <bool RELU, bool WRITE_G, bool FORK>
-__global__ void __launch_bounds__(kBlock)
+template <int MASK, bool WRITE_G, bool FORK>
+__global__ void __launch_bounds__(kBlock, (MASK == kMaskBits && !WRITE_G) ? 5 : 1)
 bn_bwd_reduce_kernel(const uint16_t* __restrict__ x, const uint16_t* __restrict__ dy, const uint16_t* __restrict__ dy2,
-                     const uint16_t* __restrict__ y, uint16_t* __restrict__ gout, const float* __restrict__ mean,
-                     float* __restrict__ ws, int64_t R, int C, int tx_log2, int64_t rpb) {
+                     const uint16_t* __restrict__ y, const uint8_t* __restrict__ mask, uint16_t* __restrict__ gout,
+                     const float* __restrict__ mean, float* __restrict__ ws, int64_t R, int C, int tx_log2,
+                     int64_t rpb) {
   constexpr int U = FORK ? kBnForkUnroll : kBnUnroll;
   __shared__ float s_red[kBlock * 16];
   __shared__ double s_grp[kBlock];
@@ -145,12 +160,13 @@
     sq[i] = 0.f;
     m[i] = active ? mean[c0 + i] : 0.f;
   }
-  auto body = [&](const bu4& xv, const bu4& dv, const bu4& bv, const bu4& yv, int64_t off) {
+  auto body = [&](const bu4& xv, const bu4& dv, const bu4& bv, const bu4& yv, uint32_t mb, int64_t off) {
     float xf[8], g[8];
     unpack8(xv, xf);
     unpack8(dv, g);
     if constexpr (FORK) fork_sum(g, bv);
-    if constexpr (RELU) relu_mask(g, yv);
+    if constexpr (MASK == kMaskY) relu_mask(g, yv);
+    if constexpr (MASK == kMaskBits) relu_mask_bits(g, mb);
     if constexpr (WRITE_G) st16(gout + off, pack8_exact(g));
 #pragma unroll
     for (int i = 0; i < 8; ++i) {
@@ -164,22 +180,27 @@
     int64_t off = r * C + c0;
     for (; r + (U - 1) * ty < r1; r += U * ty, off += U * step) {
       bu4 xv[U], dv[U], bv[U] = {}, yv[U] = {};
+      uint32_t mb[U] = {};
 #pragma unroll
       for (int k = 0; k < U; ++k) {
         xv[k] = ld16<false>(x + off + k * step);
         dv[k] = ld16<GS_BN_NT && WRITE_G>(dy + off + k * step);
         if constexpr (FORK) bv[k] = ld16<GS_BN_NT>(dy2 + off + k * step);
-        if constexpr (RELU) yv[k] = ld16<GS_BN_NT && WRITE_G>(y + off + k * step);
+        if constexpr (MASK == kMaskY) yv[k] = ld16<GS_BN_NT && WRITE_G>(y + off + k * step);
+        if constexpr (MASK == kMaskBits) mb[k] = mask[(off + k * step) >> 3];
       }
-#pragma unroll
-      for (int k = 0; k < U; ++k) body(xv[k], dv[k], bv[k], yv[k], off + k * step);
+      if constexpr (MASK == kMaskBits) __builtin_amdgcn_sched_barrier(0);
+#pragma unroll
+      for (int k = 0; k < U; ++k) body(xv[k], dv[k], bv[k], yv[k], mb[k], off + k * step);
     }
     for (; r < r1; r += ty, off += step) {
       bu4 bv = {0u, 0u, 0u, 0u}, yv = {0u, 0u, 0u, 0u};
+      uint32_t mb = 0;
       const bu4 xv = ld16<false>(x + off), dv = ld16<false>(dy + off);
       if constexpr (FORK) bv = ld16<false>(dy2 + off);
-      if constexpr (RELU) yv = ld16<false>(y + off);
-      body(xv, dv, bv, yv, off);
+      if constexpr (MASK == kMaskY) yv = ld16<false>(y + off);
+      if constexpr (MASK == kMaskBits) mb = mask[off >> 3];
+      body(xv, dv, bv, yv, mb, off);
     }
   }
   const int F = 16 << tx_log2;
@@ -206,10 +227,10 @@
   }
 }
 
-template <bool RELU>
+template <int MASK>
 __global__ void __launch_bounds__(kBlock)
 bn_bwd_dx_kernel(const uint16_t* __restrict__ x, const uint16_t* __restrict__ dy, const uint16_t* __restrict__ y,
-                 const float* __restrict__ mean, const float* __restrict__ invstd, const float* __restrict__ weight,
+                 const uint8_t* __restrict__ mask, const float* __restrict__ mean, const float* __restrict__ invstd, const float* __restrict__ weight,
                  const float* __restrict__ ws, int P, uint16_t* __restrict__ dx, float* __restrict__ gw,
                  float* __restrict__ gb, int64_t R, int C, int tx_log2, int64_t rpb, double inv_R) {
   __shared__ double s_fold[kBlock * 4];
@@ -258,11 +279,12 @@
     m1[i] = static_cast<float>(s_sum[tx_i * 16 + 2 * i] * inv_R);
     k2[i] = static_cast<float>(static_cast<double>(is) * is * s_sum[tx_i * 16 + 2 * i + 1] * inv_R);
   }
-  auto body = [&](const bu4& xv, const bu4& dv, const bu4& yv, int64_t off) {
+  auto body = [&](const bu4& xv, const bu4& dv, const bu4& yv, uint32_t mb, int64_t off) {
     float xf[8], g[8];
     unpack8(xv, xf);
     unpack8(dv, g);
-    if constexpr (RELU) relu_mask(g, yv);
+    if constexpr (MASK == kMaskY) relu_mask(g, yv);
+    if constexpr (MASK == kMaskBits) relu_mask_bits(g, mb);
 #pragma unroll
     for (int i = 0; i < 8; ++i) g[i] = a[i] * fmaf(m[i] - xf[i], k2[i], g[i] - m1[i]);
     st16(dx + off, pack8_dx(g));
@@ -274,58 +296,73 @@
   int64_t off = r * C + c0;
   for (; r + (kBnUnroll - 1) * ty < r1; r += kBnUnroll * ty, off += kBnUnroll * step) {
     bu4 xv[kBnUnroll], dv[kBnUnroll], yv[kBnUnroll] = {};
+    uint32_t mb[kBnUnroll] = {};
 #pragma unroll
     for (int k = 0; k < kBnUnroll; ++k) {
       xv[k] = ld16<GS_BN_NT>(x + off + k * step);
       dv[k] = ld16<GS_BN_NT>(dy + off + k * step);
-      if constexpr (RELU) yv[k] = ld16<GS_BN_NT>(y + off + k * step);
-    }
-#pragma unroll
-    for (int k = 0; k < kBnUnroll; ++k) body(xv[k], dv[k], yv[k], off + k * step);
+      if constexpr (MASK == kMaskY) yv[k] = ld16<GS_BN_NT>(y + off + k * step);
+      if constexpr (MASK == kMaskBits) mb[k] = mask[(off + k * step) >> 3];
+    }
+    if constexpr (MASK == kMaskBits) __builtin_amdgcn_sched_barrier(0);
+#pragma unroll
+    for (int k = 0; k < kBnUnroll; ++k) body(xv[k], dv[k], yv[k], mb[k], off + k * step);
   }
   for (; r < r1; r += ty, off += step) {
     bu4 yv = {0u, 0u, 0u, 0u};
+    uint32_t mb = 0;
     const bu4 xv = ld16<false>(x + off), dv = ld16<false>(dy + off);
-    if constexpr (RELU) yv = ld16<false>(y + off);
-    body(xv, dv, yv, off);
-  }
-}
-
+    if constexpr (MASK == kMaskY) yv = ld16<false>(y + off);
+    if constexpr (MASK == kMaskBits) mb = mask[off >> 3];
+    body(xv, dv, yv, mb, off);
+  }
+}
+
+__device__ __forceinline__ float relu1(float v) { return v > 0.f ? v : (v != v ? v : 0.f); }
+
+template <bool ADD, bool MASK>
 __global__ void __launch_bounds__(kBlock)
-add_relu_fwd_kernel(uint16_t* __restrict__ t, const uint16_t* __restrict__ id, int64_t nvec) {
+add_relu_fwd_kernel(uint16_t* __restrict__ t, const uint16_t* __restrict__ id, uint8_t* __restrict__ mask,
+                    int64_t nvec) {
   const int64_t base = static_cast<int64_t>(blockIdx.x) * (kBlock * kBnUnroll) + threadIdx.x;
-  bu4 a[kBnUnroll], b[kBnUnroll];
+  bu4 a[kBnUnroll], b[kBnUnroll] = {};
 #pragma unroll
   for (int k = 0; k < kBnUnroll; ++k) {
     const int64_t i = base + k * kBlock;
     if (i < nvec) {
       a[k] = ld16<false>(t + i * 8);
-      b[k] = ld16<false>(id + i * 8);
+      if constexpr (ADD) b[k] = ld16<false>(id + i * 8);
     }
   }
 #pragma unroll
   for (int k = 0; k < kBnUnroll; ++k) {
     const int64_t i = base + k * kBlock;
     if (i < nvec) {
-      float af[8], bf[8];
+      float af[8];
       unpack8(a[k], af);
-      unpack8(b[k], bf);
-#pragma unroll
-      for (int j = 0; j < 8; ++j) {
-        const float s = __uint_as_float(to_bf16(af[j] + bf[j]) << 16);
-        af[j] = s != s ? s : fmaxf(s, 0.f);
+      if constexpr (ADD) {
+        float bf[8];
+        unpack8(b[k], bf);
+#pragma unroll
+        for (int j = 0; j < 8; ++j) {
+          const float s = __uint_as_float(to_bf16(af[j] + bf[j]) << 16);
+          af[j] = s != s ? s : fmaxf(s, 0.f);
+        }
+      } else {
+#pragma unroll
+        for (int j = 0; j < 8; ++j) af[j] = relu1(af[j]);
       }
       st16(t + i * 8, pack8_exact(af));
-    }
-  }
-}
-
-
-__device__ __forceinline__ float relu1(float v) { return v > 0.f ? v : (v != v ? v : 0.f); }
-
+      if constexpr (MASK) mask[i] = mask_byte(af);
+    }
+  }
+}
+
+
+template <bool MASK>
 __global__ void __launch_bounds__(kBlock)
 relu_maxpool_fwd_kernel(const uint16_t* __restrict__ y, uint16_t* __restrict__ pooled, uint8_t* __restrict__ idx,
-                        int64_t nvec, int H, int W, int OH, int OW, int V) {
+                        uint8_t* __restrict__ mask, int64_t nvec, int H, int W, int OH, int OW, int V) {
   const int64_t i = static_cast<int64_t>(blockIdx.x) * kBlock + threadIdx.x;
   if (i >= nvec) return;
   const int cv = static_cast<int>(i % V);
@@ -359,6 +396,10 @@
   for (int k = 0; k < 9; ++k) {
     float f[8];
     unpack8(in[k], f);
+    if constexpr (MASK) {
+      if ((k == 4 || k == 5 || k == 7 || k == 8) && ok[k])
+        mask[((n * H + h0 + k / 3) * W + w0 + k % 3) * V + cv] = mask_byte(f);
+    }
 #pragma unroll
     for (int j = 0; j < 8; ++j) {
       const float v = relu1(f[j]);
@@ -642,12 +683,13 @@
   return GS_OK;
 }
 
-int bn_reduce(const char* who, const void* x, const void* dy, const void* dy_b, const void* y, void* g_out,
-              const float* mean, float* ws, int64_t ws_floats, int64_t R, int C, void* stream) {
+int bn_reduce(const char* who, const void* x, const void* dy, const void* dy_b, const void* y, bool bits,
+              const void* mask, void* g_out, const float* mean, float* ws, int64_t ws_floats, int64_t R, int C,
+              void* stream) {
   const std::string w(who);
   GS_TRY_RET(check_shape(R, C));
-  GS_CHECK_ARG(x && dy && mean && ws, w + ": null pointer");
-  GS_CHECK_ARG(!g_out || y || dy_b, w + ": g_out needs y");
+  GS_CHECK_ARG(x && dy && mean && ws && (!bits || mask), w + ": null pointer");
+  GS_CHECK_ARG(!g_out || y || mask || dy_b, w + ": g_out needs y");
   GS_CHECK_ARG(!dy_b || g_out, w + ": two gradients need g_out");
   GS_CHECK_ARG(aligned16(x) && aligned16(dy) && aligned16(dy_b) && aligned16(y) && aligned16(g_out) && aligned16(ws),
                w + ": pointers must be 16-byte aligned");
@@ -657,6 +699,7 @@
                      !overlap(g_out, y, bytes),
                  w + ": g_out overlaps an input");
   }
+  GS_CHECK_ARG(!overlap(g_out, R * C * 2, mask, R * C / 8), w + ": g_out overlaps the mask");
   const BnGeom g = bn_geom(R, C);
   GS_CHECK_ARG(ws_floats >= static_cast<int64_t>(g.P) * C * 2, w + ": workspace too small");
   const dim3 grid(g.ctiles, g.P), block(kBlock);
@@ -665,15 +708,19 @@
   const uint16_t* dp = static_cast<const uint16_t*>(dy);
   const uint16_t* bp = static_cast<const uint16_t*>(dy_b);
   const uint16_t* yp = static_cast<const uint16_t*>(y);
+  const uint8_t* mp = static_cast<const uint8_t*>(mask);
   uint16_t* gp = static_cast<uint16_t*>(g_out);
-#define GS_BN_REDUCE(RELU, WRITE_G, FORK)                                                                        \
-  hipLaunchKernelGGL((bn_bwd_reduce_kernel<RELU, WRITE_G, FORK>), grid, block, 0, s, xp, dp, bp, yp, gp, mean, ws, R, \
-                     C, g.tx_log2, g.rpb)
-  if (bp && yp) GS_BN_REDUCE(true, true, true);
-  else if (bp) GS_BN_REDUCE(false, true, true);
-  else if (gp) GS_BN_REDUCE(true, true, false);
-  else if (yp) GS_BN_REDUCE(true, false, false);
-  else GS_BN_REDUCE(false, false, false);
+#define GS_BN_REDUCE(MASK, WRITE_G, FORK)                                                                            \
+  hipLaunchKernelGGL((bn_bwd_reduce_kernel<MASK, WRITE_G, FORK>), grid, block, 0, s, xp, dp, bp, yp, mp, gp, mean, ws, \
+                     R, C, g.tx_log2, g.rpb)
+  if (mp && bp) GS_BN_REDUCE(kMaskBits, true, true);
+  else if (mp && gp) GS_BN_REDUCE(kMaskBits, true, false);
+  else if (mp) GS_BN_REDUCE(kMaskBits, false, false);
+  else if (bp && yp) GS_BN_REDUCE(kMaskY, true, true);
+  else if (bp) GS_BN_REDUCE(kMaskNone, true, true);
+  else if (gp) GS_BN_REDUCE(kMaskY, true, false);
+  else if (yp) GS_BN_REDUCE(kMaskY, false, false);
+  else GS_BN_REDUCE(kMaskNone, false, false);
 #undef GS_BN_REDUCE
   HIP_RET(hipGetLastError());
   return GS_OK;
@@ -684,71 +731,148 @@
 
 extern "C" int gs_bn_bwd_reduce(const void* x, const void* dy, const void* y, void* g_out, const float* mean,
                                 float* ws, int64_t ws_floats, int64_t R, int C, void* stream) {
-  return bn_reduce("gs_bn_bwd_reduce", x, dy, nullptr, y, g_out, mean, ws, ws_floats, R, C, stream);
+  return bn_reduce("gs_bn_bwd_reduce", x, dy, nullptr, y, false, nullptr, g_out, mean, ws, ws_floats, R, C, stream);
+}
+
+extern "C" int gs_bn_bwd_reduce_bits(const void* x, const void* dy, const void* mask, void* g_out, const float* mean,
+                                     float* ws, int64_t ws_floats, int64_t R, int C, void* stream) {
+  return bn_reduce("gs_bn_bwd_reduce_bits", x, dy, nullptr, nullptr, true, mask, g_out, mean, ws, ws_floats, R, C,
+                   stream);
 }
 
 extern "C" int gs_bn_bwd_reduce_fork(const void* x, const void* dy_a, const void* dy_b, const void* y, void* g_out,
                                      const float* mean, float* ws, int64_t ws_floats, int64_t R, int C,
                                      void* stream) {
-  return bn_reduce("gs_bn_bwd_reduce_fork", x, dy_a, dy_b, y, g_out, mean, ws, ws_floats, R, C, stream);
-}
-
-extern "C" int gs_bn_bwd_dx(const void* x, const void* dy, const void* y, const float* mean, const float* invstd,
-                            const float* weight, const float* ws, int64_t ws_floats, void* dx, float* grad_weight,
-                            float* grad_bias, int64_t R, int C, void* stream) {
+  return bn_reduce("gs_bn_bwd_reduce_fork", x, dy_a, dy_b, y, false, nullptr, g_out, mean, ws, ws_floats, R, C,
+                   stream);
+}
+
+extern "C" int gs_bn_bwd_reduce_fork_bits(const void* x, const void* dy_a, const void* dy_b, const void* mask,
+                                          void* g_out, const float* mean, float* ws, int64_t ws_floats, int64_t R,
+                                          int C, void* stream) {
+  return bn_reduce("gs_bn_bwd_reduce_fork_bits", x, dy_a, dy_b, nullptr, true, mask, g_out, mean, ws, ws_floats, R, C,
+                   stream);
+}
+
+namespace gs {
+namespace {
+
+int bn_dx(const std::string& w, const void* x, const void* dy, const void* y, bool bits, const void* mask,
+          const float* mean, const float* invstd, const float* weight, const float* ws, int64_t ws_floats, void* dx,
+          float* grad_weight, float* grad_bias, int64_t R, int C, void* stream) {
   GS_TRY_RET(check_shape(R, C));
-  GS_CHECK_ARG(x && dy && mean && invstd && weight && ws && dx && grad_weight && grad_bias,
-               "gs_bn_bwd_dx: null pointer");
+  GS_CHECK_ARG(x && dy && mean && invstd && weight && ws && dx && grad_weight && grad_bias && (!bits || mask),
+               w + ": null pointer");
   GS_CHECK_ARG(aligned16(x) && aligned16(dy) && aligned16(y) && aligned16(dx) && aligned16(ws),
-               "gs_bn_bwd_dx: pointers must be 16-byte aligned");
+               w + ": pointers must be 16-byte aligned");
+  GS_CHECK_ARG(!overlap(dx, R * C * 2, mask, R * C / 8), w + ": dx overlaps the mask");
   const BnGeom g = bn_geom(R, C);
-  GS_CHECK_ARG(ws_floats >= static_cast<int64_t>(g.P) * C * 2, "gs_bn_bwd_dx: workspace too small");
+  GS_CHECK_ARG(ws_floats >= static_cast<int64_t>(g.P) * C * 2, w + ": workspace too small");
   const dim3 grid(g.ctiles, g.P), block(kBlock);
   hipStream_t s = static_cast<hipStream_t>(stream);
   const uint16_t* xp = static_cast<const uint16_t*>(x);
   const uint16_t* dp = static_cast<const uint16_t*>(dy);
   const uint16_t* yp = static_cast<const uint16_t*>(y);
+  const uint8_t* mp = static_cast<const uint8_t*>(mask);
   uint16_t* op = static_cast<uint16_t*>(dx);
   const double inv_R = 1.0 / static_cast<double>(R);
-  if (yp)
-    hipLaunchKernelGGL((bn_bwd_dx_kernel<true>), grid, block, 0, s, xp, dp, yp, mean, invstd, weight, ws, g.P, op,
-                       grad_weight, grad_bias, R, C, g.tx_log2, g.rpb, inv_R);
-  else
-    hipLaunchKernelGGL((bn_bwd_dx_kernel<false>), grid, block, 0, s, xp, dp, yp, mean, invstd, weight, ws, g.P, op,
-                       grad_weight, grad_bias, R, C, g.tx_log2, g.rpb, inv_R);
+#define GS_BN_DX(MASK)                                                                                              \
+  hipLaunchKernelGGL((bn_bwd_dx_kernel<MASK>), grid, block, 0, s, xp, dp, yp, mp, mean, invstd, weight, ws, g.P, op, \
+                     grad_weight, grad_bias, R, C, g.tx_log2, g.rpb, inv_R)
+  if (mp) GS_BN_DX(kMaskBits);
+  else if (yp) GS_BN_DX(kMaskY);
+  else GS_BN_DX(kMaskNone);
+#undef GS_BN_DX
   HIP_RET(hipGetLastError());
   return GS_OK;
 }
 
-extern "C" int gs_add_relu_fwd(void* t, const void* identity, int64_t n, void* stream) {
-  GS_CHECK_ARG(t && identity && n > 0 && n % 8 == 0, "gs_add_relu_fwd: n > 0, n % 8 == 0 and pointers required");
-  GS_CHECK_ARG(aligned16(t) && aligned16(identity), "gs_add_relu_fwd: pointers must be 16-byte aligned");
+int relu_tail(const std::string& w, void* t, const void* identity, bool add, void* mask, bool bits, int64_t n,
+              void* stream) {
+  GS_CHECK_ARG(t && (!add || identity) && (!bits || mask) && n > 0 && n % 8 == 0,
+               w + ": n > 0, n % 8 == 0 and pointers required");
+  GS_CHECK_ARG(aligned16(t) && aligned16(identity), w + ": pointers must be 16-byte aligned");
+  GS_CHECK_ARG(n <= INT64_MAX / 4, w + ": n too large");
+  GS_CHECK_ARG(!overlap(mask, n / 8, t, n * 2) && !overlap(mask, n / 8, identity, n * 2),
+               w + ": the mask overlaps an activation");
   const int64_t nvec = n / 8;
   const int64_t blocks = (nvec + kBlock * kBnUnroll - 1) / (kBlock * kBnUnroll);
-  GS_CHECK_ARG(blocks <= INT_MAX, "gs_add_relu_fwd: n too large");
-  hipLaunchKernelGGL(add_relu_fwd_kernel, dim3(static_cast<unsigned>(blocks)), dim3(kBlock), 0,
-                     static_cast<hipStream_t>(stream), static_cast<uint16_t*>(t),
-                     static_cast<const uint16_t*>(identity), nvec);
+  GS_CHECK_ARG(blocks <= INT_MAX, w + ": n too large");
+  const dim3 grid(static_cast<unsigned>(blocks)), block(kBlock);
+  hipStream_t s = static_cast<hipStream_t>(stream);
+  uint16_t* tp = static_cast<uint16_t*>(t);
+  const uint16_t* ip = static_cast<const uint16_t*>(identity);
+  uint8_t* mp = static_cast<uint8_t*>(mask);
+  if (!add) hipLaunchKernelGGL((add_relu_fwd_kernel<false, true>), grid, block, 0, s, tp, ip, mp, nvec);
+  else if (bits) hipLaunchKernelGGL((add_relu_fwd_kernel<true, true>), grid, block, 0, s, tp, ip, mp, nvec);
+  else hipLaunchKernelGGL((add_relu_fwd_kernel<true, false>), grid, block, 0, s, tp, ip, mp, nvec);
   HIP_RET(hipGetLastError());
   return GS_OK;
 }
 
+int relu_maxpool(const std::string& w, const void* y, void* pooled, void* idx, void* mask, bool bits, int64_t N, int H,
+                 int W, int C, void* stream) {
+  PoolGeom g;
+  GS_TRY_RET(pool_geom(w, N, H, W, C, &g));
+  GS_CHECK_ARG(y && pooled && idx && (!bits || mask), w + ": null pointer");
+  GS_CHECK_ARG(aligned16(y) && aligned16(pooled) && aligned16(idx), w + ": pointers must be 16-byte aligned");
+  const int64_t ib = g.in_vecs * 16, ob = g.out_vecs * 16, xb = g.out_vecs * 8, mb = g.in_vecs;
+  GS_CHECK_ARG(!overlap(y, ib, pooled, ob) && !overlap(y, ib, idx, xb) && !overlap(pooled, ob, idx, xb) &&
+                   !overlap(mask, mb, y, ib) && !overlap(mask, mb, pooled, ob) && !overlap(mask, mb, idx, xb),
+               w + ": buffers overlap");
+  const dim3 grid(static_cast<unsigned>((g.out_vecs + kBlock - 1) / kBlock)), block(kBlock);
+  hipStream_t s = static_cast<hipStream_t>(stream);
+  const uint16_t* yp = static_cast<const uint16_t*>(y);
+  uint16_t* pp = static_cast<uint16_t*>(pooled);
+  uint8_t* ip = static_cast<uint8_t*>(idx);
+  uint8_t* mp = static_cast<uint8_t*>(mask);
+  if (mp)
+    hipLaunchKernelGGL((relu_maxpool_fwd_kernel<true>), grid, block, 0, s, yp, pp, ip, mp, g.out_vecs, H, W, g.OH, g.OW,
+                       C / 8);
+  else
+    hipLaunchKernelGGL((relu_maxpool_fwd_kernel<false>), grid, block, 0, s, yp, pp, ip, mp, g.out_vecs, H, W, g.OH,
+                       g.OW, C / 8);
+  HIP_RET(hipGetLastError());
+  return GS_OK;
+}
+
+}
+}
+
+extern "C" int gs_bn_bwd_dx(const void* x, const void* dy, const void* y, const float* mean, const float* invstd,
+                            const float* weight, const float* ws, int64_t ws_floats, void* dx, float* grad_weight,
+                            float* grad_bias, int64_t R, int C, void* stream) {
+  return bn_dx("gs_bn_bwd_dx", x, dy, y, false, nullptr, mean, invstd, weight, ws, ws_floats, dx, grad_weight,
+               grad_bias, R, C, stream);
+}
+
+extern "C" int gs_bn_bwd_dx_bits(const void* x, const void* dy, const void* mask, const float* mean,
+                                 const float* invstd, const float* weight, const float* ws, int64_t ws_floats,
+                                 void* dx, float* grad_weight, float* grad_bias, int64_t R, int C, void* stream) {
+  return bn_dx("gs_bn_bwd_dx_bits", x, dy, nullptr, true, mask, mean, invstd, weight, ws, ws_floats, dx, grad_weight,
+               grad_bias, R, C, stream);
+}
+
+extern "C" int gs_add_relu_fwd(void* t, const void* identity, int64_t n, void* stream) {
+  return relu_tail("gs_add_relu_fwd", t, identity, true, nullptr, false, n, stream);
+}
+
+extern "C" int gs_add_relu_mask_fwd(void* t, const void* identity, void* mask, int64_t n, void* stream) {
+  return relu_tail("gs_add_relu_mask_fwd", t, identity, true, mask, true, n, stream);
+}
+
+extern "C" int gs_relu_mask_fwd(void* t, void* mask, int64_t n, void* stream) {
+  return relu_tail("gs_relu_mask_fwd", t, nullptr, false, mask, true, n, stream);
+}
+
 extern "C" int gs_relu_maxpool_fwd(const void* y, void* pooled, void* idx, int64_t N, int H, int W, int C,
                                    void* stream) {
-  const std::string w("gs_relu_maxpool_fwd");
-  PoolGeom g;
-  GS_TRY_RET(pool_geom(w, N, H, W, C, &g));
-  GS_CHECK_ARG(y && pooled && idx, w + ": null pointer");
-  GS_CHECK_ARG(aligned16(y) && aligned16(pooled) && aligned16(idx), w + ": pointers must be 16-byte aligned");
-  const int64_t ib = g.in_vecs * 16, ob = g.out_vecs * 16, xb = g.out_vecs * 8;
-  GS_CHECK_ARG(!overlap(y, ib, pooled, ob) && !overlap(y, ib, idx, xb) && !overlap(pooled, ob, idx, xb),
-               w + ": buffers overlap");
-  const unsigned blocks = static_cast<unsigned>((g.out_vecs + kBlock - 1) / kBlock);
-  hipLaunchKernelGGL(relu_maxpool_fwd_kernel, dim3(blocks), dim3(kBlock), 0, static_cast<hipStream_t>(stream),
-                     static_cast<const uint16_t*>(y), static_cast<uint16_t*>(pooled), static_cast<uint8_t*>(idx),
-                     g.out_vecs, H, W, g.OH, g.OW, C / 8);
-  HIP_RET(hipGetLastError());
-  return GS_OK;
+  return relu_maxpool("gs_relu_maxpool_fwd", y, pooled, idx, nullptr, false, N, H, W, C, stream);
+}
+
+extern "C" int gs_relu_maxpool_mask_fwd(const void* y, void* pooled, void* idx, void* mask, int64_t N, int H, int W,
+                                        int C, void* stream) {
+  return relu_maxpool("gs_relu_maxpool_mask_fwd", y, pooled, idx, mask, true, N, H, W, C, stream);
 }
 
 extern "C" int gs_maxpool_bwd(const void* d_a, const void* d_b, const void* idx, void* dx, int64_t N, int H, int W,
diff --git a/distributed_training_amd/fused_bn.py b/distributed_training_amd/fused_bn.py
--- a/distributed_training_amd/fused_bn.py
+++ b/distributed_training_amd/fused_bn.py
@@ -20,6 +20,10 @@
     if P is None:
         P = _partials[(R, C)] = L.check(L.lib().gs_bn_bwd_partials(R, C), "gs_bn_bwd_partials")
     return P
+
+
+def _mask_bits() -> bool:
+    return os.environ.get("GSYNC_BN_MASK", "1") != "0"
 
 
 def _eligible(bn, x, relu, residual) -> bool:
@@ -100,14 +104,24 @@
             x, weight, bias, bn.running_mean, bn.running_var, True, momentum, bn.eps, torch.backends.cudnn.enabled)
         if not y.is_contiguous(memory_format=_CL):
             raise RuntimeError("fused_bn: batch_norm returned a layout other than its channels_last input's")
-        if residual is not None:
+        mask = None
+        if relu and _mask_bits():
+            mask = torch.empty(y.numel() // 8, dtype=torch.uint8, device=y.device)
+        if residual is not None and mask is not None:
+            L.check(L.lib().gs_add_relu_mask_fwd(y.data_ptr(), residual.data_ptr(), mask.data_ptr(), y.numel(),
+                                                 L.stream_ptr(y.device)), "gs_add_relu_mask_fwd")
+        elif residual is not None:
             L.check(L.lib().gs_add_relu_fwd(y.data_ptr(), residual.data_ptr(), y.numel(), L.stream_ptr(y.device)),
                     "gs_add_relu_fwd")
+        elif mask is not None:
+            L.check(L.lib().gs_relu_mask_fwd(y.data_ptr(), mask.data_ptr(), y.numel(), L.stream_ptr(y.device)),
+                    "gs_relu_mask_fwd")
         elif relu:
             torch.relu_(y)
         ctx.relu = relu
+        ctx.bits = mask is not None
         ctx.has_residual = residual is not None
-        ctx.save_for_backward(x, weight, mean, invstd, y if relu else None)
+        ctx.save_for_backward(x, weight, mean, invstd, mask if mask is not None else (y if relu else None))
         if fork:
             ctx.set_materialize_grads(False)
             return y, y.view_as(y)
@@ -133,24 +147,28 @@
         gb = torch.empty_like(weight)
         lib, stream = L.lib(), L.stream_ptr(x.device)
         yp = y.data_ptr() if ctx.relu else None
+        bits = ctx.bits
         g = None
         if dy_b is not None:
             g = torch.empty_like(x)
-            L.check(lib.gs_bn_bwd_reduce_fork(x.data_ptr(), dy.data_ptr(), dy_b.data_ptr(), yp, g.data_ptr(),
-                                              mean.data_ptr(), ws.data_ptr(), ws.numel(), R, C, stream),
-                    "gs_bn_bwd_reduce_fork")
+            fn = "gs_bn_bwd_reduce_fork_bits" if bits else "gs_bn_bwd_reduce_fork"
+            L.check(getattr(lib, fn)(x.data_ptr(), dy.data_ptr(), dy_b.data_ptr(), yp, g.data_ptr(), mean.data_ptr(),
+                                     ws.data_ptr(), ws.numel(), R, C, stream), fn)
             dy, yp = g, None
         elif ctx.has_residual:
             g = torch.empty_like(x)
-            L.check(lib.gs_bn_bwd_reduce(x.data_ptr(), dy.data_ptr(), yp, g.data_ptr(), mean.data_ptr(),
-                                         ws.data_ptr(), ws.numel(), R, C, stream), "gs_bn_bwd_reduce")
+            fn = "gs_bn_bwd_reduce_bits" if bits else "gs_bn_bwd_reduce"
+            L.check(getattr(lib, fn)(x.data_ptr(), dy.data_ptr(), yp, g.data_ptr(), mean.data_ptr(), ws.data_ptr(),
+                                     ws.numel(), R, C, stream), fn)
             dy, yp = g, None
         else:
-            L.check(lib.gs_bn_bwd_reduce(x.data_ptr(), dy.data_ptr(), yp, None, mean.data_ptr(), ws.data_ptr(),
-                                         ws.numel(), R, C, stream), "gs_bn_bwd_reduce")
-        L.check(lib.gs_bn_bwd_dx(x.data_ptr(), dy.data_ptr(), yp, mean.data_ptr(), invstd.data_ptr(),
+            fn = "gs_bn_bwd_reduce_bits" if bits else "gs_bn_bwd_reduce"
+            L.check(getattr(lib, fn)(x.data_ptr(), dy.data_ptr(), yp, None, mean.data_ptr(), ws.data_ptr(),
+                                     ws.numel(), R, C, stream), fn)
+        fn = "gs_bn_bwd_dx_bits" if bits and yp is not None else "gs_bn_bwd_dx"
+        L.check(getattr(lib, fn)(x.data_ptr(), dy.data_ptr(), yp, mean.data_ptr(), invstd.data_ptr(),
                                  weight.data_ptr(), ws.data_ptr(), ws.numel(), dx.data_ptr(), gw.data_ptr(),
-                                 gb.data_ptr(), R, C, stream), "gs_bn_bwd_dx")
+                                 gb.data_ptr(), R, C, stream), fn)
         return dx, gw, gb, g if ctx.has_residual else None, None, None, None, None
 
 
@@ -166,8 +184,15 @@
         OH, OW = (H - 1) // 2 + 1, (W - 1) // 2 + 1
         out = torch.empty((N, C, OH, OW), dtype=y.dtype, device=y.device, memory_format=_CL)
         idx = torch.empty((N, OH, OW, C), dtype=torch.uint8, device=y.device)
-        L.check(L.lib().gs_relu_maxpool_fwd(y.data_ptr(), out.data_ptr(), idx.data_ptr(), N, H, W, C,
-                                            L.stream_ptr(y.device)), "gs_relu_maxpool_fwd")
+        ctx.bits = _mask_bits()
+        if ctx.bits:
+            mask = torch.empty(y.numel() // 8, dtype=torch.uint8, device=y.device)
+            L.check(L.lib().gs_relu_maxpool_mask_fwd(y.data_ptr(), out.data_ptr(), idx.data_ptr(), mask.data_ptr(), N,
+                                                     H, W, C, L.stream_ptr(y.device)), "gs_relu_maxpool_mask_fwd")
+            y = mask
+        else:
+            L.check(L.lib().gs_relu_maxpool_fwd(y.data_ptr(), out.data_ptr(), idx.data_ptr(), N, H, W, C,
+                                                L.stream_ptr(y.device)), "gs_relu_maxpool_fwd")
         ctx.save_for_backward(x, weight, mean, invstd, y, idx)
         if fork:
             ctx.set_materialize_grads(False)
@@ -196,11 +221,13 @@
         dx = torch.empty_like(x)
         gw = torch.empty_like(weight)
         gb = torch.empty_like(weight)
-        L.check(lib.gs_bn_bwd_reduce(x.data_ptr(), dy.data_ptr(), y.data_ptr(), None, mean.data_ptr(), ws.data_ptr(),
-                                     ws.numel(), R, C, stream), "gs_bn_bwd_reduce")
-        L.check(lib.gs_bn_bwd_dx(x.data_ptr(), dy.data_ptr(), y.data_ptr(), mean.data_ptr(), invstd.data_ptr(),
+        fn = "gs_bn_bwd_reduce_bits" if ctx.bits else "gs_bn_bwd_reduce"
+        L.check(getattr(lib, fn)(x.data_ptr(), dy.data_ptr(), y.data_ptr(), None, mean.data_ptr(), ws.data_ptr(),
+                                 ws.numel(), R, C, stream), fn)
+        fn = "gs_bn_bwd_dx_bits" if ctx.bits else "gs_bn_bwd_dx"
+        L.check(getattr(lib, fn)(x.data_ptr(), dy.data_ptr(), y.data_ptr(), mean.data_ptr(), invstd.data_ptr(),
                                  weight.data_ptr(), ws.data_ptr(), ws.numel(), dx.data_ptr(), gw.data_ptr(),
-                                 gb.data_ptr(), R, C, stream), "gs_bn_bwd_dx")
+                                 gb.data_ptr(), R, C, stream), fn)
         return dx, gw, gb, None, None, None
 
 
diff --git a/include/gsync.h b/include/gsync.h
--- a/include/gsync.h
+++ b/include/gsync.h
@@ -231,6 +231,17 @@
 int gs_relu_maxpool_fwd(const void* y, void* pooled, void* idx, int64_t N, int H, int W, int C, void* stream);
 int gs_maxpool_bwd(const void* d_a, const void* d_b, const void* idx, void* dx, int64_t N, int H, int W, int C,
                    void* stream);
+int gs_relu_mask_fwd(void* t, void* mask, int64_t n, void* stream);
+int gs_add_relu_mask_fwd(void* t, const void* identity, void* mask, int64_t n, void* stream);
+int gs_relu_maxpool_mask_fwd(const void* y, void* pooled, void* idx, void* mask, int64_t N, int H, int W, int C,
+                             void* stream);
+int gs_bn_bwd_reduce_bits(const void* x, const void* dy, const void* mask, void* g_out, const float* mean, float* ws,
+                          int64_t ws_floats, int64_t R, int C, void* stream);
+int gs_bn_bwd_reduce_fork_bits(const void* x, const void* dy_a, const void* dy_b, const void* mask, void* g_out,
+                               const float* mean, float* ws, int64_t ws_floats, int64_t R, int C, void* stream);
+int gs_bn_bwd_dx_bits(const void* x, const void* dy, const void* mask, const float* mean, const float* invstd,
+                      const float* weight, const float* ws, int64_t ws_floats, void* dx, float* grad_weight,
+                      float* grad_bias, int64_t R, int C, void* stream);
 
 int gs_bn_infer_act(const void* x, const void* residual, const float* running_mean, const float* running_var,
                     const float* weight, const float* bias, double eps, int relu, void* y, int64_t R, int C,
```

Result: faster. 7051, median of 6 (+2.4%).
